# michaelfeil/skyjo_rl

Hardware: AMD Instinct MI355X
Metric: env-steps/sec (whole node) at 65 536 parallel 3-player games (higher is better)
Workload: dtype int8

## Files before the change

### skyjo_rl_amd/csrc/skyjo_capi.hip

```cpp
#include <hip/hip_runtime.h>
#include <hip/hip_ext.h>

#include <cstdio>
#include <cstdlib>
#include <atomic>
#include <cmath>
#include <cstring>
#include <new>
#include <string>
#include <vector>

#include "skyjo_device.h"
#include "skyjo_policy.h"
#include "skyjo_targets.h"
#include "skyjo_batches.h"

#ifdef SK_DIAG
static const char *sk_diag_env(const char *name) { return getenv(name); }
#else
static inline const char *sk_diag_env(const char *) { return nullptr; }
#endif

namespace {

// ... 44 lines not shown
  int cycle_s = 0;
};

enum class InFlight {
  None,
  ListRun,
  Planned,
  Dealing
};

enum class DealRun : int {
  ListBeside = 0,
  ListInline = 1,
  ScanInline = 2,
  Planned = 3
};
constexpr int deal_interval_default(int num_players, DealForm form, int cycle_s) {
  switch (form) {
    case DealForm::OneKernel:
      if (cycle_s >= 4) return num_players >= 3 ? 64 : 56;
      return num_players >= 4 ? 104 : (num_players == 3 ? 80 : 56);
    case DealForm::TwoStreamsPipelined: return num_players >= 3 ? 80 : 56;
    case DealForm::TwoStreamsScanPublish: return num_players >= 3 ? 64 : 48;
    default: return num_players >= 3 ? 88 : 64;
  }
}

}

struct skyjo_vec_mlp {
  SkMlpDev net{};
  void *blob = nullptr;
  int device_id = 0, obs_dim = 0;
};

struct skyjo_vec {
  uint64_t generation = 0;
  skyjo_vec_config cfg{};
  SkParams P{};
  size_t G = 0;
  size_t lds_bytes = 0, lds_tile = 0;
  size_t lds_rollout = 0, lds_step = 0;
  bool seeded = false;
  int pending_iters = 0;
  int deal_every_iters = 64;
  bool auto_interval = true;
  int interval_default = 64, calm_runs = 0;
  uint32_t health_seen = 0;
  uint32_t *health_host = nullptr;
  DealRequests req;
  DealForm form = DealForm::InlineScan;
  bool one_kernel_capable = false;
  int cycle_s = SK_CYCLE_MAX_S;
  size_t lds_cycle = 0, lds_cycle_step = 0;
  uint32_t cycle_deal_arg = 0;
  hipStream_t deal_stream = nullptr;
  hipEvent_t ev_scan = nullptr, ev_dealt = nullptr;
  InFlight inflight = InFlight::None;
  uint32_t inflight_tag = 0;
  int list_sel = 0;
  uint32_t deal_tag = 0;
  uint64_t iter = 0;
  uint64_t iters_total = 0;
  bool fast_host = false, raw_valid = false;
  bool host_spin = true;
  bool raw_export = false;
  uint8_t *hm_block = nullptr;
  int32_t *hm_actions = nullptr;
  uint8_t *hm_mask = nullptr, *hm_records = nullptr, *hm_raw = nullptr;
  int32_t *hm_actions_d = nullptr;
  uint8_t *hm_mask_d = nullptr, *hm_records_d = nullptr, *hm_raw_d = nullptr;
  int raw_stride = 0;
  uint32_t host_seq = 0;
  uint32_t cycle_seq = 0;
  int ncu = 256;
  int max_cycles = 0;
  bool rec_planar_all = false;
  bool rec_planar = false;
  int32_t *d_actions = nullptr;
  uint8_t *d_records = nullptr;
  uint8_t *d_mask = nullptr;
  void *sel_scratch = nullptr;
  size_t sel_blocks = 0;
  std::vector<std::pair<void *, size_t>> allocs;
  std::vector<void *> owned;
  uint8_t *arena = nullptr;
  size_t arena_off = 0;
  int arena_mode = 0;
  bool profile = false;
  std::vector<std::pair<hipEvent_t, hipEvent_t>> ev[SKYJO_PROF_KERNELS];
};

struct skyjo_vec_snapshot {
  const skyjo_vec *owner = nullptr;
  uint64_t owner_generation = 0;
  std::vector<size_t> array_bytes;
  int device_id = 0;
  void *blob = nullptr;
  size_t bytes = 0;
  int pending_iters = 0, deal_every_iters = 0, calm_runs = 0, list_sel = 0;
  bool auto_interval = true;
  uint32_t health_seen = 0, deal_tag = 0, health[2] = {0, 0};
  uint64_t iter = 0, iters_total = 0;
};

namespace {

int dev_error_check(const skyjo_vec *h) {
  if (h->health_host && (h->health_host[2] & SK_ERR_DEAL_TIMEOUT))
    return fail(SKYJO_E_DEVICE, "a step kernel gave up waiting for the dealing kernel that should run beside it (SKYJO_OPT_OVERLAP): "
                                "results since then are void; switch the option off or re-seed");
  return SKYJO_OK;
}

int dev_error_fetch(skyjo_vec *h, hipStream_t s) {
  uint32_t err = 0;
  HIPCHK(hipMemcpyAsync(&err, h->P.dev_error, sizeof(err), hipMemcpyDeviceToHost, s));
  HIPCHK(hipStreamSynchronize(s));
  h->health_host[2] |= err;
  return dev_error_check(h);
}

template <class T>
int dalloc(skyjo_vec *h, T **out, size_t count, bool zero = true) {
  const size_t bytes = count * sizeof(T);
  void *p = nullptr;
  if (h->arena_mode) {
    const size_t al = bytes >= ((size_t)1 << 20) ? ((size_t)2 << 20) : 256;
    const size_t off = (h->arena_off + al - 1) & ~(al - 1);
    h->arena_off = off + bytes;
    if (h->arena_mode == 1) {
      *out = nullptr;
      return SKYJO_OK;
    }
    p = h->arena + off;
  } else {
    HIPCHK(hipMalloc(&p, bytes));
    h->owned.push_back(p);
  }
  if (zero) HIPCHK(hipMemset(p, 0, bytes));
  h->allocs.emplace_back(p, bytes);
  *out = (T *)p;
  return SKYJO_OK;
}

int prof_events(skyjo_vec *h, int kernel, hipEvent_t *a, hipEvent_t *b) {
  *a = *b = nullptr;
  if (!h->profile) return SKYJO_OK;
  HIPCHK(hipEventCreate(a));
  HIPCHK(hipEventCreate(b));
  h->ev[kernel].emplace_back(*a, *b);
  return SKYJO_OK;
}

constexpr uint32_t kDealLds = SK_TILE * (SK_DECK_STRIDE + SK_STG_STRIDE);
constexpr int fixed_players(int n) { return n >= 2 && n <= 4 ? n : 0; }

template <class Fn>
struct KernelRow {
  int key;
  Fn fn;
};
constexpr int kernel_key(int players, bool indirect = false, bool planar = false, bool policy = false) {
  return players | indirect << 4 | planar << 5 | policy << 6;
}
template <class Fn, size_t K>
Fn find_kernel(const KernelRow<Fn> (&table)[K], int key) {
  for (const KernelRow<Fn> &r : table)
    if (r.key == key) return r.fn;
  return nullptr;
}

constexpr KernelRow<decltype(&k_deal<2>)> kDealKernels[] = {{2, k_deal<2>}, {3, k_deal<3>}, {4, k_deal<4>}, {0, k_deal<0>}};

#define SK_ROW(I, NP, PL) {kernel_key(NP, I, PL), k_cycle<I, NP, PL>}
#define SK_ROWS(I, PL) SK_ROW(I, 2, PL), SK_ROW(I, 3, PL), SK_ROW(I, 4, PL)
constexpr KernelRow<decltype(&k_cycle<true, 2, false>)> kCycleKernels[] = {SK_ROWS(true, false), SK_ROWS(true, true), SK_ROWS(false, true), SK_ROWS(false, false)};
#undef SK_ROWS
#undef SK_ROW

#define SK_ROW(I, Pol, NP, PL) {kernel_key(NP, I, PL, Pol), k_step<I, Pol, NP, PL>}
#define SK_ROWS(I, Pol) SK_ROW(I, Pol, 2, false), SK_ROW(I, Pol, 3, false), SK_ROW(I, Pol, 4, false), SK_ROW(I, Pol, 0, false)
constexpr KernelRow<decltype(&k_step<true, true, 2>)> kStepKernels[] = {SK_ROW(true, false, 2, true), SK_ROW(true, false, 3, true), SK_ROW(true, false, 4, true),
                                                                        SK_ROWS(true, true), SK_ROWS(true, false), SK_ROWS(false, true), SK_ROWS(false, false)};
#undef SK_ROWS
#undef SK_ROW

int launch_deal_kernel(skyjo_vec *h, hipStream_t ds, DealRun run, int be_read = -1) {
  hipEvent_t e0, e1;
  int rc;
  h->P.be_read = be_read >= 0 ? (uint32_t)be_read : (h->P.deal_tag & 1u);
  if ((rc = prof_events(h, 2, &e0, &e1))) return rc;
  const int np = fixed_players(h->P.L.N);
  hipExtLaunchKernelGGL(find_kernel(kDealKernels, kernel_key(np)), dim3(h->P.tiles), dim3(SK_TILE), np ? kDealLds : (uint32_t)(h->lds_tile + 16384), ds, e0, e1, 0, h->P,
                        h->list_sel, (int)run);
  HIPCHK(hipGetLastError());
  return SKYJO_OK;
}

int flush_planned(skyjo_vec *h, hipStream_t s) {
  if (h->inflight != InFlight::Planned) return SKYJO_OK;
  const uint32_t keep = h->P.deal_tag;
  h->P.deal_tag = h->inflight_tag;
  h->inflight = InFlight::Dealing;
  const int rc = launch_deal_kernel(h, s, DealRun::Planned, (int)((h->cycle_seq - 1u) & 1u));
  h->P.deal_tag = keep;
  return rc;
}

int publish_deals(skyjo_vec *h, hipStream_t s) {
  int rc = flush_planned(h, s);
  if (rc) return rc;
  if (h->inflight == InFlight::None) return SKYJO_OK;
  if (uses_deal_stream(h->form)) HIPCHK(hipStreamWaitEvent(s, h->ev_dealt, 0));
  hipEvent_t e0, e1;
  if ((rc = prof_events(h, 3, &e0, &e1))) return rc;
  if (h->inflight == InFlight::ListRun) {
    hipExtLaunchKernelGGL(k_publish, dim3(64), dim3(256), 0, s, e0, e1, 0, h->P, h->list_sel);
  } else {
    const int G = h->P.tiles * SK_TILE;
    hipExtLaunchKernelGGL(k_publish_all, dim3((G + 255) / 256), dim3(256), 0, s, e0, e1, 0, h->P);
  }
  HIPCHK(hipGetLastError());
  h->inflight = InFlight::None;
// ... 179 lines not shown
      const char *e = sk_diag_env("SKYJO_OVERLAP");
      one = prefer_one && !e;
      beside = !one && (e ? atoi(e) != 0 : P.tiles <= 768);
    }
  }
  h->form = one      ? DealForm::OneKernel
            : beside ? (h->req.unpipelined ? DealForm::TwoStreamsScanPublish : DealForm::TwoStreamsPipelined)
                     : (h->req.inline_work_list ? DealForm::InlineWorkList : DealForm::InlineScan);
  h->interval_default = deal_interval_default(N, h->form, h->cycle_s);
  if (h->auto_interval) h->deal_every_iters = h->interval_default;
}

int change_form(skyjo_vec *h, const DealRequests &req) {
  HIPCHK(hipDeviceSynchronize());
  int rc = publish_deals(h, nullptr);
  if (rc) return rc;
  HIPCHK(hipDeviceSynchronize());
  h->req = req;
  resolve_form(h);
  return SKYJO_OK;
}

}

extern "C" {

const char *skyjo_vec_last_error(void) { return g_err.c_str(); }
int skyjo_vec_abi_version(void) { return SKYJO_ABI_VERSION; }

int skyjo_vec_create(const skyjo_vec_config *cfg, skyjo_vec **out) {
  if (!cfg || !out) return fail(SKYJO_E_INVALID, "null argument");
  *out = nullptr;
  if (cfg->abi_version != SKYJO_ABI_VERSION) return fail(SKYJO_E_INVALID, "abi_version mismatch");
  if (cfg->num_envs <= 0) return fail(SKYJO_E_INVALID, "num_envs must be > 0");
  if (cfg->num_players <= 0 || cfg->num_players > SKYJO_MAX_PLAYERS)
    return fail(SKYJO_E_INVALID, "Skyjo can be played from 1 up to 8 (recommended) / 12 (theoretical) players");
  if (cfg->rng_mode != SKYJO_RNG_MT19937 && cfg->rng_mode != SKYJO_RNG_PHILOX)
    return fail(SKYJO_E_INVALID, "unknown rng_mode");
  int ndev = 0;
  if (hipGetDeviceCount(&ndev) != hipSuccess || ndev <= 0)
    return fail(SKYJO_E_NOGPU, "no HIP device visible: this library has no CPU fallback");
  if (cfg->device_id < 0 || cfg->device_id >= ndev) return fail(SKYJO_E_INVALID, "device_id out of range");
  hipDeviceProp_t prop;
  HIPCHK(hipGetDeviceProperties(&prop, cfg->device_id));
  if (strncmp(prop.gcnArchName, "gfx950", 6) != 0 && !sk_diag_env("SKYJO_ALLOW_ANY_GPU"))
    return fail(SKYJO_E_NOGPU, std::string("device is ") + prop.gcnArchName + ", kernels are built for gfx950");
  DevGuard guard_(cfg->device_id);

  skyjo_vec *h = new (std::nothrow) skyjo_vec();
  if (!h) return fail(SKYJO_E_INVALID, "out of host memory");
  h->cfg = *cfg;
  h->generation = ++g_generation;
  SkParams &P = h->P;
  P.L = sk_make_layout(cfg->num_players, cfg->observe_indirect);
  P.B = cfg->num_envs;
  P.tiles = (cfg->num_envs + SK_TILE - 1) / SK_TILE;
  P.rng_mode = cfg->rng_mode;
  P.auto_reset = cfg->auto_reset ? 1 : 0;
  P.score_penalty = cfg->score_penalty, P.mean_reward = cfg->mean_reward;
  P.reward_refunded = cfg->reward_refunded, P.illegal_reward = cfg->illegal_reward;
  P.game_id0 = cfg->game_id0;
  P.spin_log2 = 22, P.debug_deal_delay = 0;
  h->G = (size_t)P.tiles * SK_TILE;
  h->lds_tile = (size_t)P.L.chunks * 1024;
  h->lds_bytes = h->lds_tile + (size_t)SK_TILE * (P.L.indirect ? 64 : P.L.rec_bytes + 16) + (size_t)SK_ACC_KINDS * cfg->num_players * 512 +
                 (cfg->num_players < 8 ? (size_t)cfg->num_players * 1024 : 0);
  const bool fixed_n = cfg->num_players >= 2 && cfg->num_players <= 4;
  h->lds_step = fixed_n ? h->lds_tile + (size_t)SK_TILE * (P.L.indirect ? 64 : P.L.rec_bytes + 16) : h->lds_bytes;
  h->lds_rollout = fixed_n ? h->lds_step + (size_t)cfg->num_players * 1024 : h->lds_bytes;
  if (const char *e = sk_diag_env("SKYJO_LDS_PAD"))
    h->lds_bytes += (size_t)atoi(e), h->lds_rollout += (size_t)atoi(e), h->lds_step += (size_t)atoi(e);
  const size_t rec16 = (size_t)P.tiles * P.L.chunks * SK_TILE;
  if ((uint64_t)SK_BANK * rec16 * 16 >= (1ull << 32)) {
    delete h;
    return fail(SKYJO_E_INVALID, "num_envs too large for one handle");
  }
  int rc = SKYJO_OK;
  const size_t N = (size_t)cfg->num_players;
  auto carve = [&]() -> int {
    int rc = SKYJO_OK;
    if (cfg->rng_mode == SKYJO_RNG_MT19937 && (rc = dalloc(h, &P.mt, h->G * 624 + 16, false)  )) {
      return rc;
    }
    if ((rc = dalloc(h, &P.state, rec16)) || (rc = dalloc(h, &P.spare, SK_BANK * rec16)) ||
        (rc = dalloc(h, &P.spare_ready, SK_BANK * h->G)) || (rc = dalloc(h, &P.bank_head, h->G)) ||
        (rc = dalloc(h, &P.busy, h->G)) || (rc = dalloc(h, &P.cancel, h->G)) || (rc = dalloc(h, &P.done_flag, h->G)) || (rc = dalloc(h, &P.plan_tag, h->G)) || (rc = dalloc(h, &P.plan_ep, h->G)) ||
        (rc = dalloc(h, &P.deal_list, 2 * h->G)) || (rc = dalloc(h, &P.deal_ep, 2 * h->G)) ||
        (rc = dalloc(h, &P.deal_count, 2)) || (rc = dalloc(h, &P.bank_empty, 2)) ||
        (rc = dalloc(h, &P.mt_idx, (1 + SK_BANK) * h->G)) || (rc = dalloc(h, &P.seeds, h->G)) ||
        (rc = dalloc(h, &P.deals_consumed, h->G)) || (rc = dalloc(h, &P.rewards, h->G * N)) ||
        (rc = dalloc(h, &P.scores, h->G * N)) || (rc = dalloc(h, &P.done, h->G)) ||
        (rc = dalloc(h, &P.acc_tile, (size_t)P.tiles * SK_ACC_KINDS * SKYJO_MAX_PLAYERS)) || (rc = dalloc(h, &P.dev_error, 1)) ||
        (rc = dalloc(h, &P.counters, 1)) || (rc = dalloc(h, &P.tile_counters, (size_t)P.tiles * 8)) || (rc = dalloc(h, &P.stamps, (size_t)P.tiles * 32))) {
      return rc;
    }
    return SKYJO_OK;
  };
  h->arena_mode = 1, h->arena_off = 0;
  (void)carve();
  {
    const size_t two_mb = (size_t)2 << 20, total = h->arena_off + two_mb;
    void *raw = nullptr;
    if (hipMalloc(&raw, total) != hipSuccess) {
      skyjo_vec_destroy(h);
      return fail(SKYJO_E_DEVICE, "hipMalloc failed for the engine's arrays");
    }
    h->owned.push_back(raw);
    h->arena = (uint8_t *)(((uintptr_t)raw + two_mb - 1) & ~(uintptr_t)(two_mb - 1));
  }
  h->arena_mode = 2, h->arena_off = 0;
  rc = carve();
  h->arena_mode = 0;
  if (rc) {
    skyjo_vec_destroy(h);
    return rc;
  }
  int prio_least = 0, prio_greatest = 0;
  (void)hipDeviceGetStreamPriorityRange(&prio_least, &prio_greatest);
  if (hipStreamCreateWithPriority(&h->deal_stream, hipStreamNonBlocking, prio_least) != hipSuccess ||
      hipEventCreateWithFlags(&h->ev_scan, hipEventDisableTiming) != hipSuccess ||
      hipEventCreateWithFlags(&h->ev_dealt, hipEventDisableTiming) != hipSuccess) {
    skyjo_vec_destroy(h);
    return fail(SKYJO_E_DEVICE, "cannot create the dealing stream / events");
  }
  {
    void *dp = nullptr;
    if (hipHostMalloc((void **)&h->health_host, 4 * sizeof(uint32_t), hipHostMallocMapped) != hipSuccess ||
        hipHostGetDevicePointer(&dp, h->health_host, 0) != hipSuccess) {
      skyjo_vec_destroy(h);
      return fail(SKYJO_E_DEVICE, "cannot map the bank-health word");
    }
    h->health_host[0] = h->health_host[1] = h->health_host[2] = h->health_host[3] = 0;
    P.health_host = (volatile uint32_t *)dp;
  }
  h->raw_stride = (int)((P.L.state_bytes + 16 * cfg->num_players + 8 + 15) & ~15);
  if (h->G <= 4096) {
    const size_t a = (h->G * 4 + 255) & ~(size_t)255, m = (h->G + 255) & ~(size_t)255, r = (h->G * (size_t)P.L.rec_bytes + 255) & ~(size_t)255,
                 w = h->G * (size_t)h->raw_stride;
    void *dp = nullptr;
    if (hipHostMalloc((void **)&h->hm_block, a + m + r + w, hipHostMallocMapped) == hipSuccess &&
        hipHostGetDevicePointer(&dp, h->hm_block, 0) == hipSuccess) {
      memset(h->hm_block, 0, a + m + r + w);
      uint8_t *d = (uint8_t *)dp;
      h->hm_actions = (int32_t *)h->hm_block, h->hm_mask = h->hm_block + a, h->hm_records = h->hm_block + a + m, h->hm_raw = h->hm_block + a + m + r;
      h->hm_actions_d = (int32_t *)d, h->hm_mask_d = d + a, h->hm_records_d = d + a + m, h->hm_raw_d = d + a + m + r;
      h->fast_host = !sk_diag_env("SKYJO_NO_FAST_HOST");
      h->host_spin = !sk_diag_env("SKYJO_NO_SPIN");
      h->raw_export = h->fast_host && P.tiles <= 4 && !sk_diag_env("SKYJO_NO_RAW_EXPORT");
    }
  }
  h->ncu = prop.multiProcessorCount > 0 ? prop.multiProcessorCount : 256;
  if (const char *e = sk_diag_env("SKYJO_FUSED_SCAN")) h->req.inline_work_list = atoi(e) == 0;
  if (const char *e = sk_diag_env("SKYJO_PIPELINED")) h->req.unpipelined = atoi(e) == 0;
  resolve_form(h);
  if (const char *e = sk_diag_env("SKYJO_DEAL_INTERVAL")) {
    const int v = atoi(e);
    if (v >= 1 && v <= 1024) h->deal_every_iters = v, h->auto_interval = false;
  }
  *out = h;
  return SKYJO_OK;
}

int skyjo_vec_destroy(skyjo_vec *h) {
  if (!h) return SKYJO_OK;
  GUARD(h);
  (void)hipDeviceSynchronize();
  if (h->deal_stream) (void)hipStreamDestroy(h->deal_stream);
  if (h->ev_scan) (void)hipEventDestroy(h->ev_scan);
  if (h->ev_dealt) (void)hipEventDestroy(h->ev_dealt);
  for (void *p : h->owned) (void)hipFree(p);
  if (h->sel_scratch) (void)hipFree(h->sel_scratch);
  for (auto &v : h->ev)
    for (auto &e : v) (void)hipEventDestroy(e.first), (void)hipEventDestroy(e.second);
  if (h->health_host) (void)hipHostFree(h->health_host);
  if (h->hm_block) (void)hipHostFree(h->hm_block);
  delete h;
  return SKYJO_OK;
}

int skyjo_vec_get_info(const skyjo_vec *h, skyjo_vec_info *out) {
  if (!h || !out) return fail(SKYJO_E_INVALID, "null argument");
  const SkLayout &L = h->P.L;
  out->num_envs = h->P.B, out->num_players = L.N, out->obs_dim = L.D, out->record_bytes = L.rec_bytes;
  out->mask_offset = L.Dp, out->meta_offset = L.Dp + 26, out->state_bytes = L.state_bytes, out->tile_games = SK_TILE;
  return SKYJO_OK;
}

int skyjo_vec_seed(skyjo_vec *h, const uint64_t *seeds_host, uint64_t base_seed, void *stream) {
  if (!h) return fail(SKYJO_E_INVALID, "null handle");
  hipStream_t s = (hipStream_t)stream;
  GUARD(h);
  h->raw_valid = false;
  uint64_t *d_seeds = nullptr;
  if (seeds_host) {
    HIPCHK(hipMalloc((void **)&d_seeds, sizeof(uint64_t) * (size_t)h->P.B));
    HIPCHK(hipMemcpyAsync(d_seeds, seeds_host, sizeof(uint64_t) * (size_t)h->P.B, hipMemcpyHostToDevice, s));
  }
  HIPCHK(hipDeviceSynchronize());
  HIPCHK(hipMemsetAsync(h->P.done, 0, h->G, s));
  HIPCHK(hipMemsetAsync(h->P.dev_error, 0, sizeof(uint32_t), s));
  h->health_host[2] = 0;
  int rc0;
  if ((rc0 = publish_deals(h, s))) return rc0;
  hipLaunchKernelGGL(k_seed, dim3((h->P.B + 255) / 256), dim3(256), 0, s, h->P, (const uint64_t *)d_seeds, base_seed, 0,
                     h->P.B);
  HIPCHK(hipGetLastError());
  int rc;
  h->inflight = InFlight::None;
  if ((rc = start_deals(h, s)) || (rc = publish_deals(h, s))) return rc;
  h->seeded = true;
  if ((rc = skyjo_vec_reset(h, nullptr, nullptr, stream))) return rc;
  for (int k = 1; k < SK_BANK; k++)
    if ((rc = start_deals(h, s)) || (rc = publish_deals(h, s))) return rc;
  if (d_seeds) {
    HIPCHK(hipStreamSynchronize(s));
    HIPCHK(hipFree(d_seeds));
  }
  h->iter = 0;
  return skyjo_vec_reset_counters(h, stream);
}

static int ensure_scratch(skyjo_vec *h);

int skyjo_vec_seed_one(skyjo_vec *h, int32_t game, uint64_t value, void *stream) {
  if (!h || game < 0 || game >= h->P.B) return fail(SKYJO_E_INVALID, "bad argument");
  if (!h->seeded) return fail(SKYJO_E_STATE, "skyjo_vec_seed must be called first");
  GUARD(h);
  h->raw_valid = false;
  hipStream_t s = (hipStream_t)stream;
  int rc;
  if ((rc = ensure_scratch(h)) || (rc = publish_deals(h, s))) return rc;
  uint64_t *d_seed = (uint64_t *)h->d_actions;
  HIPCHK(hipMemcpyAsync(d_seed, &value, sizeof(value), hipMemcpyHostToDevice, s));
  HIPCHK(hipStreamSynchronize(s));
  hipLaunchKernelGGL(k_seed, dim3(1), dim3(64), 0, s, h->P, (const uint64_t *)d_seed, (uint64_t)0, (int)game, 1);
  HIPCHK(hipGetLastError());
  if ((rc = start_deals(h, s)) || (rc = publish_deals(h, s))) return rc;
  HIPCHK(hipMemsetAsync(h->d_mask, 0, h->G, s));
  const uint8_t one = 1;
  HIPCHK(hipMemcpyAsync(h->d_mask + game, &one, 1, hipMemcpyHostToDevice, s));
  HIPCHK(hipStreamSynchronize(s));
  if ((rc = skyjo_vec_reset(h, h->d_mask, nullptr, stream))) return rc;
  for (int k = 1; k < SK_BANK; k++)
    if ((rc = start_deals(h, s)) || (rc = publish_deals(h, s))) return rc;
  return SKYJO_OK;
}

int skyjo_vec_snapshot_create(skyjo_vec *h, skyjo_vec_snapshot **out, void *stream) {
  if (!h || !out) return fail(SKYJO_E_INVALID, "null argument");
  if (!h->seeded) return fail(SKYJO_E_STATE, "skyjo_vec_seed must be called first");
  GUARD(h);
  hipStream_t s = (hipStream_t)stream;
  int rc;
  if ((rc = publish_deals(h, s))) return rc;
  HIPCHK(hipDeviceSynchronize());
  if ((rc = dev_error_fetch(h, s))) return rc;
  skyjo_vec_snapshot *sn = new (std::nothrow) skyjo_vec_snapshot();
  if (!sn) return fail(SKYJO_E_INVALID, "out of host memory");
  sn->owner = h, sn->owner_generation = h->generation, sn->device_id = h->cfg.device_id;
  for (auto &a : h->allocs) sn->bytes += (a.second + 255) & ~(size_t)255, sn->array_bytes.push_back(a.second);
  if (hipMalloc(&sn->blob, sn->bytes) != hipSuccess) {
    delete sn;
    return fail(SKYJO_E_DEVICE, "hipMalloc failed for the snapshot");
  }
  size_t off = 0;
  for (auto &a : h->allocs) {
    hipError_t e = hipMemcpyAsync((uint8_t *)sn->blob + off, a.first, a.second, hipMemcpyDeviceToDevice, s);
    if (e != hipSuccess) {
      (void)hipFree(sn->blob);
      delete sn;
      return fail(SKYJO_E_DEVICE, std::string("snapshot copy: ") + hipGetErrorString(e));
    }
    off += (a.second + 255) & ~(size_t)255;
  }
  if (hipError_t e = hipStreamSynchronize(s); e != hipSuccess) {
    (void)hipFree(sn->blob);
    delete sn;
    return fail(SKYJO_E_DEVICE, std::string("snapshot copy: ") + hipGetErrorString(e));
  }
  sn->pending_iters = h->pending_iters, sn->deal_every_iters = h->deal_every_iters, sn->calm_runs = h->calm_runs;
  sn->list_sel = h->list_sel, sn->auto_interval = h->auto_interval, sn->health_seen = h->health_seen;
  sn->deal_tag = h->deal_tag, sn->iter = h->iter, sn->iters_total = h->iters_total;
  sn->health[0] = h->health_host[0], sn->health[1] = h->health_host[1];
  *out = sn;
  return SKYJO_OK;
}

int skyjo_vec_snapshot_restore(skyjo_vec *h, const skyjo_vec_snapshot *sn, void *stream) {
  if (!h || !sn) return fail(SKYJO_E_INVALID, "null argument");
  if (sn->owner != h || sn->owner_generation != h->generation)
    return fail(SKYJO_E_INVALID, "the snapshot was taken from another handle");
  if (sn->array_bytes.size() > h->allocs.size()) return fail(SKYJO_E_INVALID, "the snapshot does not fit the handle's arrays");
  for (size_t k = 0; k < sn->array_bytes.size(); k++)
    if (sn->array_bytes[k] != h->allocs[k].second) return fail(SKYJO_E_INVALID, "the snapshot does not fit the handle's arrays");
  GUARD(h);
  hipStream_t s = (hipStream_t)stream;
  int rc;
  if ((rc = publish_deals(h, s))) return rc;
  HIPCHK(hipDeviceSynchronize());
  size_t off = 0;
  for (size_t k = 0; k < sn->array_bytes.size(); k++) {
    const auto &a = h->allocs[k];
    HIPCHK(hipMemcpyAsync(a.first, (const uint8_t *)sn->blob + off, a.second, hipMemcpyDeviceToDevice, s));
    off += (a.second + 255) & ~(size_t)255;
  }
  HIPCHK(hipStreamSynchronize(s));
  h->pending_iters = sn->pending_iters, h->deal_every_iters = sn->deal_every_iters, h->calm_runs = sn->calm_runs;
  h->list_sel = sn->list_sel, h->auto_interval = sn->auto_interval, h->health_seen = sn->health_seen;
  h->deal_tag = sn->deal_tag, h->P.deal_tag = sn->deal_tag, h->iter = sn->iter, h->iters_total = sn->iters_total;
  h->health_host[0] = sn->health[0], h->health_host[1] = sn->health[1];
  h->health_host[2] = 0;
  h->inflight = InFlight::None;
  h->raw_valid = false;
  return SKYJO_OK;
}

int skyjo_vec_snapshot_bytes(const skyjo_vec_snapshot *sn, size_t *bytes_out) {
  if (!sn || !bytes_out) return fail(SKYJO_E_INVALID, "null argument");
  *bytes_out = sn->bytes;
  return SKYJO_OK;
}

int skyjo_vec_snapshot_destroy(skyjo_vec_snapshot *sn) {
  if (!sn) return SKYJO_OK;
  DevGuard guard_(sn->device_id);
  (void)hipFree(sn->blob);
  delete sn;
  return SKYJO_OK;
}

static int reset_impl(skyjo_vec *h, const uint8_t *mask, void *records_out, hipStream_t s, uint8_t *raw_out, int planar = 0) {
  int rc;
  h->raw_valid = false;
  if ((rc = publish_deals(h, s))) return rc;
  dim3 grid(h->P.tiles), block(SK_TILE);
  if (h->P.L.indirect)
    hipLaunchKernelGGL((k_reset<true>), grid, block, h->lds_bytes, s, h->P, mask, (uint8_t *)records_out, raw_out, h->raw_stride, planar);
  else
    hipLaunchKernelGGL((k_reset<false>), grid, block, h->lds_bytes, s, h->P, mask, (uint8_t *)records_out, raw_out, h->raw_stride, 0);
  HIPCHK(hipGetLastError());
  if ((rc = start_deals(h, s))) return rc;
  return publish_deals(h, s);
}

int skyjo_vec_reset(skyjo_vec *h, const uint8_t *mask, void *records_out, void *stream) {
  if (!h) return fail(SKYJO_E_INVALID, "null handle");
  GUARD(h);
  if (!h->seeded) return fail(SKYJO_E_STATE, "skyjo_vec_seed must be called first");
  return reset_impl(h, mask, records_out, (hipStream_t)stream, nullptr, h->rec_planar_all ? 1 : 0);
}

static int step_once(skyjo_vec *h, const int32_t *actions, void *records_out, double *end_rew, uint8_t *end_flag, hipStream_t s,
                     uint8_t *raw_out = nullptr, bool planar_out = false) {
  const bool due = h->pending_iters + 1 >= h->deal_every_iters;
  if (due && plans_ahead(h)) plan_cycle(h);
  int rc = launch_step(h, s, false, actions, (uint8_t *)records_out, nullptr, 1, 0, end_rew, end_flag, raw_out, 0, planar_out && records_out);
  if (rc) return rc;
  return due ? start_due_deals(h, s) : SKYJO_OK;
}

int skyjo_vec_step(skyjo_vec *h, const int32_t *actions, void *records_out, void *stream) {
  if (!h || !actions) return fail(SKYJO_E_INVALID, "null argument");
  GUARD(h);
  if (!h->seeded) return fail(SKYJO_E_STATE, "skyjo_vec_seed must be called first");
  return step_once(h, actions, records_out, nullptr, nullptr, (hipStream_t)stream, nullptr, h->rec_planar_all);
}

int skyjo_vec_step_collect(skyjo_vec *h, const int32_t *actions, void *records_out, double *final_rewards_out,
                           uint8_t *episode_end_out, void *stream) {
  if (!h || !actions || !final_rewards_out || !episode_end_out) return fail(SKYJO_E_INVALID, "null argument");
  GUARD(h);
  if (!h->seeded) return fail(SKYJO_E_STATE, "skyjo_vec_seed must be called first");
  return step_once(h, actions, records_out, final_rewards_out, episode_end_out, (hipStream_t)stream, nullptr, h->rec_planar_all);
}

static int model_check(skyjo_vec *h, const skyjo_vec_mlp *policy, const skyjo_vec_mlp *value, int32_t T, const skyjo_vec_rollout_buffers *b) {
  if (!h || !policy || !b || T < 0 || !b->records || !b->actions) return fail(SKYJO_E_INVALID, "skyjo_vec_model_rollout: bad argument");
  if (value && !b->values) return fail(SKYJO_E_INVALID, "skyjo_vec_model_rollout: a value net needs a values buffer");
  if ((b->final_rewards == nullptr) != (b->episode_end == nullptr))
    return fail(SKYJO_E_INVALID, "skyjo_vec_model_rollout: final_rewards and episode_end go together");
  if (!h->seeded) return fail(SKYJO_E_STATE, "skyjo_vec_seed must be called first");
  if (policy->net.out_dim != SKYJO_NUM_ACTIONS) return fail(SKYJO_E_INVALID, "the policy net needs 26 outputs");
  if (policy->device_id != h->cfg.device_id || policy->obs_dim != h->P.L.D || !h->P.L.indirect)
    return fail(SKYJO_E_INVALID, "the policy net must live on the engine's device and take the engine's (indirect) observation");
  if (value && (policy->obs_dim != value->obs_dim || policy->device_id != value->device_id || policy->net.split != value->net.split))
    return fail(SKYJO_E_INVALID, "policy and value net must share the observation size, the precision and the device");
  return SKYJO_OK;
}
// ... 31 lines not shown
}

int skyjo_vec_rollout(skyjo_vec *h, int32_t iters, uint64_t policy_seed, void *records_out, int32_t *actions_out,
                      void *stream) {
  if (!h || iters < 0) return fail(SKYJO_E_INVALID, "bad argument");
  GUARD(h);
  if (!h->seeded) return fail(SKYJO_E_STATE, "skyjo_vec_seed must be called first");
  hipStream_t s = (hipStream_t)stream;
  uint8_t *rec = (uint8_t *)records_out;
  const bool planar = h->rec_planar;
  if (planar && rec && h->form != DealForm::OneKernel)
    return fail(SKYJO_E_STATE, "SKYJO_OPT_RECORD_LAYOUT = tile-planar needs the one-kernel dealing form (SKYJO_OPT_OVERLAP 3)");
  for (int done = 0; done < iters;) {
    int n = iters - done < kMaxRolloutChunk ? iters - done : kMaxRolloutChunk;
    const int due = h->deal_every_iters - h->pending_iters;
    if (n > due) n = due > 0 ? due : 1;
    const bool run_due = h->pending_iters + n >= h->deal_every_iters, planned = plans_ahead(h);
    int cycles = 1;
    if (h->form == DealForm::OneKernel && planned && run_due && h->pending_iters == 0) {
      const int cap = h->max_cycles > 0 ? h->max_cycles : kMaxCyclesPerLaunch;
      cycles = (iters - done) / h->deal_every_iters;
      cycles = cycles < 1 ? 1 : (cycles > cap ? cap : cycles);
      n = cycles * h->deal_every_iters;
    }
    if (run_due && planned) {
      plan_cycle(h);
      const uint32_t first = h->deal_tag;
      for (int c = 1; c < cycles; c++) next_deal_tag(h, false);
      h->P.plan_new_tag = first;
    }
    int rc = launch_step(h, s, true, nullptr, rec, actions_out, n, policy_seed, nullptr, nullptr, nullptr, cycles > 1 ? h->deal_every_iters : 0);
    if (rc) return rc;
    done += n;
    if (run_due && (rc = start_due_deals(h, s))) return rc;
    if (rec) rec += (size_t)n * (planar ? h->G : (size_t)h->P.B) * h->P.L.rec_bytes;
    if (actions_out) actions_out += (size_t)n * h->P.B;
  }
  return SKYJO_OK;
}

static int observe_impl(skyjo_vec *h, const int32_t *players, void *records_out, void *stream, int planar) {
  if (!h || !records_out) return fail(SKYJO_E_INVALID, "null argument");
  GUARD(h);
  if (!h->seeded) return fail(SKYJO_E_STATE, "skyjo_vec_seed must be called first");
  dim3 grid(h->P.tiles), block(SK_TILE);
  hipStream_t s = (hipStream_t)stream;
  if (h->P.L.indirect)
    hipLaunchKernelGGL((k_observe<true>), grid, block, h->lds_bytes, s, h->P, players, (uint8_t *)records_out, planar);
  else
    hipLaunchKernelGGL((k_observe<false>), grid, block, h->lds_bytes, s, h->P, players, (uint8_t *)records_out, 0);
  HIPCHK(hipGetLastError());
  return SKYJO_OK;
}
int skyjo_vec_observe(skyjo_vec *h, const int32_t *players, void *records_out, void *stream) {
  return observe_impl(h, players, records_out, stream, h && h->rec_planar_all ? 1 : 0);
}

static int unpack_impl(skyjo_vec *h, const void *records, int64_t n, int8_t *obs, int8_t *mask, uint8_t *agent, uint8_t *phase, uint8_t *done,
                       uint8_t *status, void *stream, int planar) {
  if (!h || !records || n < 0) return fail(SKYJO_E_INVALID, "bad argument");
  GUARD(h);
  if (n == 0) return SKYJO_OK;
  long long total = n * (long long)(h->P.L.D + 26);
  int blocks = (int)((total + 255) / 256);
  if (blocks > 4096) blocks = 4096;
  hipLaunchKernelGGL(k_unpack, dim3(blocks), dim3(256), 0, (hipStream_t)stream, h->P.L, (const uint8_t *)records,
                     (long long)n, obs, mask, agent, phase, done, status, planar);
  HIPCHK(hipGetLastError());
  return SKYJO_OK;
}

int skyjo_vec_unpack(skyjo_vec *h, const void *records, int64_t n, int8_t *obs, int8_t *mask, uint8_t *agent,
                     uint8_t *phase, uint8_t *done, uint8_t *status, void *stream) {
  return unpack_impl(h, records, n, obs, mask, agent, phase, done, status, stream, 0);
}

int skyjo_vec_unpack_tiles(skyjo_vec *h, const void *records, int64_t n_tiles, int8_t *obs, int8_t *mask, uint8_t *agent,
                           uint8_t *phase, uint8_t *done, uint8_t *status, void *stream) {
  return unpack_impl(h, records, n_tiles * SK_TILE, obs, mask, agent, phase, done, status, stream, 1);
}

const double *skyjo_vec_rewards_ptr(const skyjo_vec *h) { return h ? h->P.rewards : nullptr; }
const double *skyjo_vec_scores_ptr(const skyjo_vec *h) { return h ? h->P.scores : nullptr; }
const uint8_t *skyjo_vec_done_ptr(const skyjo_vec *h) { return h ? h->P.done : nullptr; }

int skyjo_vec_sample_actions_layout(skyjo_vec *h, const void *records, int32_t layout, const float *logits, int64_t n, uint64_t seed,
                                    uint64_t ticket, int32_t no_masking, int32_t *actions_out, float *logp_out,
                                    float *uniform_out, void *stream) {
  if (!h || !records || !logits || !actions_out || n < 0) return fail(SKYJO_E_INVALID, "null argument");
  if (layout != SKYJO_REC_ROW_MAJOR && layout != SKYJO_REC_TILE_PLANAR) return fail(SKYJO_E_INVALID, "layout must be SKYJO_REC_ROW_MAJOR or SKYJO_REC_TILE_PLANAR");
  GUARD(h);
  if (n == 0) return SKYJO_OK;
  const int64_t blocks = (n + SK_SAMPLE_BLOCK - 1) / SK_SAMPLE_BLOCK;
  hipLaunchKernelGGL(k_sample, dim3((unsigned)blocks), dim3(SK_SAMPLE_BLOCK), 0, (hipStream_t)stream, h->P.L,
                     (const uint8_t *)records, logits, (long long)n, seed, ticket, h->P.game_id0, (int)no_masking,
                     actions_out, logp_out, uniform_out, (int)(layout == SKYJO_REC_TILE_PLANAR));
  HIPCHK(hipGetLastError());
  return SKYJO_OK;
}
int skyjo_vec_sample_actions(skyjo_vec *h, const void *records, const float *logits, int64_t n, uint64_t seed,
                             uint64_t ticket, int32_t no_masking, int32_t *actions_out, float *logp_out,
                             float *uniform_out, void *stream) {
  return skyjo_vec_sample_actions_layout(h, records, SKYJO_REC_ROW_MAJOR, logits, n, seed, ticket, no_masking, actions_out, logp_out, uniform_out,
                                         stream);
}

int skyjo_vec_mlp_create(int32_t device_id, int32_t obs_dim, int32_t out_dim, int32_t precision, const float *w1, const float *b1,
                         const float *w2, const float *b2, const float *w3, const float *b3, skyjo_vec_mlp **out) {
  if (!out || !w1 || !b1 || !w2 || !b2 || !w3 || !b3) return fail(SKYJO_E_INVALID, "null argument");
  if (obs_dim < 1 || obs_dim > SKP_IN - 1 || out_dim < 1 || out_dim > SKP_OUT)
    return fail(SKYJO_E_INVALID, "skyjo_vec_mlp: obs_dim must be 1..31 and out_dim 1..32");
  if (precision != SKYJO_MLP_BF16 && precision != SKYJO_MLP_FP32) return fail(SKYJO_E_INVALID, "skyjo_vec_mlp: unknown precision");
  int ndev = 0;
  if (hipGetDeviceCount(&ndev) != hipSuccess || device_id < 0 || device_id >= ndev) return fail(SKYJO_E_INVALID, "device_id out of range");
  DevGuard guard_(device_id);
  auto bf16 = [](float f) {
    uint32_t u;
    memcpy(&u, &f, 4);
    u += 0x7fffu + ((u >> 16) & 1u);
    return (uint16_t)(u >> 16);
  };
  auto bf16_to_float = [](uint16_t b) {
    const uint32_t u = (uint32_t)b << 16;
    float f;
    memcpy(&f, &u, 4);
    return f;
  };
  auto bf16_lo = [&](float f) {
    const uint32_t hi = (uint32_t)bf16(f) << 16;
    float fh;
    memcpy(&fh, &hi, 4);
    return bf16(f - fh);
  };
  const bool split = precision == SKYJO_MLP_FP32;
  auto acc_k = [](int ks, int hh, int j) { return 32 * (ks >> 1) + 16 * (ks & 1) + 8 * (j >> 2) + 4 * hh + (j & 3); };
  const int H = SKP_HIDDEN;
  const size_t e1 = (size_t)8 * 2 * 64 * 8, e2 = (size_t)8 * 16 * 64 * 8, e3 = (size_t)16 * 64 * 8;
  std::vector<uint16_t> f1(e1), f2(e2), f3(e3), g1(split ? e1 : 0), g2(split ? e2 : 0), g3(split ? e3 : 0);
  std::vector<float> c2((size_t)H), c3((size_t)64 * 16);
  for (int u = 0; u < 8; u++)
    for (int l = 0; l < 64; l++) {
      const int m = 32 * u + (l & 31), hh = l >> 5;
      for (int s = 0; s < 2; s++)
        for (int j = 0; j < 8; j++) {
          const int k = 16 * s + 8 * hh + j;
          const float v = SKP_SCALE * (k < obs_dim ? w1[(size_t)m * obs_dim + k] : (k == SKP_IN - 1 ? b1[m] : 0.f));
          const size_t at = (((size_t)u * 2 + s) * 64 + l) * 8 + j;
          f1[at] = bf16(v);
          if (split) g1[at] = bf16_lo(v);
        }
      for (int ks = 0; ks < 16; ks++)
        for (int j = 0; j < 8; j++) {
          const float v = SKP_SCALE * w2[(size_t)m * H + acc_k(ks, hh, j)];
          const size_t at = (((size_t)u * 16 + ks) * 64 + l) * 8 + j;
          f2[at] = split ? bf16(v) : bf16(-2.0f * v);
          if (split) g2[at] = bf16_lo(v);
        }
    }
  for (int l = 0; l < 64; l++) {
    const int m = l & 31, hh = l >> 5;
    for (int ks = 0; ks < 16; ks++)
      for (int j = 0; j < 8; j++) {
        const float v = m < out_dim ? w3[(size_t)m * H + acc_k(ks, hh, j)] : 0.f;
        const size_t at = ((size_t)ks * 64 + l) * 8 + j;
        f3[at] = split ? bf16(v) : bf16(-2.0f * v);
        if (split) g3[at] = bf16_lo(v);
      }
// ... 269 lines not shown
int skyjo_vec_get_state(skyjo_vec *h, int32_t game, skyjo_game_state *o, void *stream) {
  if (!h || !o || game < 0 || game >= h->P.B) return fail(SKYJO_E_INVALID, "bad argument");
  GUARD(h);
  hipStream_t s = (hipStream_t)stream;
  const SkLayout &L = h->P.L;
  if (h->raw_valid) {
    const uint8_t *raw = h->hm_raw + (size_t)game * h->raw_stride;
    decode_state(L, raw, o);
    const double *d = (const double *)(raw + L.state_bytes);
    if (o->done) {
      memcpy(o->rewards, d, sizeof(double) * L.N);
      if (o->is_terminated) memcpy(o->final_score, d + L.N, sizeof(double) * L.N);
    }
    return dev_error_check(h);
  }
  std::vector<uint8_t> r;
  int rc = fetch_record(h, h->P.state, game, r, s);
  if (rc) return rc;
  decode_state(L, r.data(), o);
  if (o->done) {
    HIPCHK(hipMemcpyAsync(o->rewards, h->P.rewards + (size_t)game * L.N, sizeof(double) * L.N, hipMemcpyDeviceToHost, s));
    if (o->is_terminated)
      HIPCHK(hipMemcpyAsync(o->final_score, h->P.scores + (size_t)game * L.N, sizeof(double) * L.N,
                            hipMemcpyDeviceToHost, s));
    HIPCHK(hipStreamSynchronize(s));
  }
  return dev_error_check(h);
}

int skyjo_vec_set_state(skyjo_vec *h, int32_t game, const skyjo_game_state *in, void *stream) {
  if (!h || !in || game < 0 || game >= h->P.B) return fail(SKYJO_E_INVALID, "bad argument");
  GUARD(h);
  if (!h->seeded) return fail(SKYJO_E_STATE, "skyjo_vec_seed must be called first");
  h->raw_valid = false;
  const SkLayout &L = h->P.L;
  if (in->n_draw < 0 || in->n_disc < 0 || in->n_draw + in->n_disc > SK_NCARDS)
    return fail(SKYJO_E_INVALID, "pile sizes out of range");
  if (in->expected_player >= L.N || in->expected_phase > 1) return fail(SKYJO_E_INVALID, "bad expected action");
  hipStream_t s = (hipStream_t)stream;
  std::vector<uint8_t> r((size_t)L.state_bytes, 0);
  int ms = 1 << 30, mh = 1 << 30;
  for (int p = 0; p < L.N; p++) {
    int sum = 0, hid = 0;
    for (int k = 0; k < 12; k++) {
      int8_t c = in->players_cards[p][k];
      int m = in->players_masked[p][k];
      if (c < -2 && !(m == 0 && c == SKYJO_REFUNDED)) return fail(SKYJO_E_INVALID, "card value out of range");
      if (c > 12) return fail(SKYJO_E_INVALID, "card value out of range");
      int8_t v = m == 2 ? (int8_t)SKYJO_HAND_NONE : (m == 0 ? (int8_t)SKYJO_REFUNDED : c);
      r[sk_pb(L, p) + PB_CARDS + k] = (uint8_t)(m == 0 ? (int8_t)SKYJO_REFUNDED : c);
      r[sk_pb(L, p) + PB_VIS + k] = (uint8_t)v;
      if (m == 1) {
        sum += c;
        if (!L.indirect) r[H_HIST + 2 + c]++;
      }
      if (m == 2) hid++;
    }
    int16_t s16 = (int16_t)sum;
    memcpy(&r[sk_pb(L, p) + PB_SUM], &s16, 2);
    r[sk_pb(L, p) + PB_HIDDEN] = (uint8_t)hid;
    r[sk_pb(L, p) + PB_REFUNDED] = (uint8_t)in->num_refunded[p];
    uint16_t pl = (uint16_t)in->num_placed[p];
    memcpy(&r[sk_pb(L, p) + PB_PLACED], &pl, 2);
    ms = sum < ms ? sum : ms, mh = hid < mh ? hid : mh;
  }
  for (int k = 0; k < in->n_draw; k++) r[L.off_pile + k] = (uint8_t)in->drawpile[k];
  for (int k = 0; k < in->n_disc; k++) {
    int8_t c = in->discard_pile[k];
    if (c < -2 || c > 12) return fail(SKYJO_E_INVALID, "discard value out of range");
    r[L.off_pile + SK_NCARDS - 1 - k] = (uint8_t)c;
    r[H_HIST + 2 + c]++;
  }
  r[H_PHASE] = in->expected_phase, r[H_PLAYER] = in->expected_player;
  r[H_FLAGS] = F_VALID | (in->is_terminated ? (F_TERMINATED | F_DONE) : 0) | (in->done ? F_DONE : 0);
  r[H_STATUS] = in->status;
  r[H_NDRAW] = (uint8_t)in->n_draw, r[H_NDISC] = (uint8_t)in->n_disc, r[H_ROLE] = 0;
  memcpy(&r[H_EPLEN], &in->episode_steps, 2);
  r[H_RESH] = (uint8_t)(in->reshuffles > 255 ? 255 : in->reshuffles);
  memcpy(&r[H_EPISODE], &in->episode, 4);
  r[H_MINSUM] = (uint8_t)(int8_t)(ms < 127 ? ms : 127);
  r[H_MINHID] = (uint8_t)mh;
  r[H_TOP] = in->n_disc ? (uint8_t)in->discard_pile[in->n_disc - 1] : (uint8_t)(int8_t)-3;
  r[H_HAND] = (uint8_t)in->hand_card;
  HIPCHK(hipMemcpyAsync(&r[H_BANK], h->P.bank_head + game, 1, hipMemcpyDeviceToHost, s));
  HIPCHK(hipStreamSynchronize(s));
  uint8_t *dst = (uint8_t *)(h->P.state + ((size_t)(game / SK_TILE) * L.chunks) * SK_TILE + game % SK_TILE);
  HIPCHK(hipMemcpy2DAsync(dst, SK_TILE * 16, r.data(), 16, 16, L.chunks, hipMemcpyHostToDevice, s));
  uint8_t dn = (r[H_FLAGS] & F_DONE) ? 1 : 0;
  HIPCHK(hipMemcpyAsync(h->P.done + game, &dn, 1, hipMemcpyHostToDevice, s));
  if (dn) {
    HIPCHK(hipMemcpyAsync(h->P.rewards + (size_t)game * L.N, in->rewards, sizeof(double) * L.N, hipMemcpyHostToDevice, s));
    HIPCHK(hipMemcpyAsync(h->P.scores + (size_t)game * L.N, in->final_score, sizeof(double) * L.N,
                          hipMemcpyHostToDevice, s));
  }
  HIPCHK(hipStreamSynchronize(s));
  return SKYJO_OK;
}

int skyjo_vec_seed_raw(skyjo_vec *h, int32_t game, uint32_t value, void *stream) {
  if (!h || game < 0 || game >= h->P.B) return fail(SKYJO_E_INVALID, "bad argument");
  GUARD(h);
  if (!h->seeded) return fail(SKYJO_E_STATE, "skyjo_vec_seed must be called first");
  if (h->P.rng_mode != SKYJO_RNG_MT19937) return fail(SKYJO_E_STATE, "seed_raw needs the MT19937 mode");
  h->raw_valid = false;
  hipStream_t s = (hipStream_t)stream;
  int rc;
  if ((rc = publish_deals(h, s))) return rc;
  hipLaunchKernelGGL(k_seed_raw, dim3(1), dim3(64), 0, s, h->P, game, value);
  HIPCHK(hipGetLastError());
  if ((rc = start_deals(h, s))) return rc;
  return publish_deals(h, s);
}

int skyjo_vec_rng_set_state(skyjo_vec *h, int32_t game, const uint32_t *key_host, int32_t pos, void *stream) {
  if (!h || !key_host || game < 0 || game >= h->P.B || pos < 0 || pos > 624) return fail(SKYJO_E_INVALID, "bad argument");
  GUARD(h);
  if (!h->seeded) return fail(SKYJO_E_STATE, "skyjo_vec_seed must be called first");
  if (h->P.rng_mode != SKYJO_RNG_MT19937 || !h->req.no_bank)
    return fail(SKYJO_E_STATE, "skyjo_vec_rng_set_state needs the MT19937 mode and SKYJO_OPT_NO_BANK (episodes dealt ahead would belong to the old stream)");
  hipStream_t s = (hipStream_t)stream;
  const int32_t packed = pos >= 624 ? 0 : (pos | ((624 - pos) << 16));
  HIPCHK(hipMemcpyAsync(h->P.mt + (size_t)game * 624, key_host, 624 * sizeof(uint32_t), hipMemcpyHostToDevice, s));
  HIPCHK(hipMemcpyAsync(h->P.mt_idx + game, &packed, sizeof(packed), hipMemcpyHostToDevice, s));
  HIPCHK(hipStreamSynchronize(s));
  return SKYJO_OK;
}

int skyjo_vec_rng_get_state(skyjo_vec *h, int32_t game, uint32_t *key_out_host, int32_t *pos_out_host, void *stream) {
  if (!h || !key_out_host || !pos_out_host || game < 0 || game >= h->P.B) return fail(SKYJO_E_INVALID, "bad argument");
  GUARD(h);
  if (!h->seeded) return fail(SKYJO_E_STATE, "skyjo_vec_seed must be called first");
  if (h->P.rng_mode != SKYJO_RNG_MT19937 || !h->req.no_bank)
    return fail(SKYJO_E_STATE, "skyjo_vec_rng_get_state needs the MT19937 mode and SKYJO_OPT_NO_BANK");
  hipStream_t s = (hipStream_t)stream;
  int32_t packed = 0;
  HIPCHK(hipMemcpyAsync(key_out_host, h->P.mt + (size_t)game * 624, 624 * sizeof(uint32_t), hipMemcpyDeviceToHost, s));
  HIPCHK(hipMemcpyAsync(&packed, h->P.mt_idx + game, sizeof(packed), hipMemcpyDeviceToHost, s));
  HIPCHK(hipStreamSynchronize(s));
  int idx = packed & 0xffff, ahead = packed >> 16;
  if (idx >= 624) idx = 0;
  if (idx + ahead > 624) return fail(SKYJO_E_STATE, "the stream's regenerated window wraps: not a numpy state (cannot happen without a bank)");
  if (idx == 0 && ahead == 0) {
    *pos_out_host = 624;
    return SKYJO_OK;
  }
  uint32_t *mt = key_out_host;
  for (int i = idx + ahead; i < 624; i++) {
    const uint32_t y = (mt[i] & 0x80000000u) | (mt[i + 1 == 624 ? 0 : i + 1] & 0x7fffffffu);
    mt[i] = mt[i + 397 >= 624 ? i + 397 - 624 : i + 397] ^ (y >> 1) ^ ((y & 1u) ? 0x9908b0dfu : 0u);
  }
  *pos_out_host = idx;
  return SKYJO_OK;
}

int skyjo_vec_profile(skyjo_vec *h, int enable, double ms_out[SKYJO_PROF_KERNELS], int64_t launches_out[SKYJO_PROF_KERNELS]) {
  if (!h) return fail(SKYJO_E_INVALID, "null handle");
  GUARD(h);
  HIPCHK(hipDeviceSynchronize());
  for (int k = 0; k < SKYJO_PROF_KERNELS; k++) {
    double tot = 0;
    int64_t cnt = 0;
    for (auto &p : h->ev[k]) {
      float ms = 0.f;
      if (hipEventElapsedTime(&ms, p.first, p.second) == hipSuccess) tot += ms, cnt++;
      (void)hipEventDestroy(p.first);
      (void)hipEventDestroy(p.second);
    }
    h->ev[k].clear();
    if (ms_out) ms_out[k] = tot;
    if (launches_out) launches_out[k] = cnt;
  }
  h->profile = enable != 0;
// ... 115 lines not shown
    h->P.host_seq = 0;
    if (rc) return rc;
    bool arrived = false;
    if (spin) {
      const volatile uint32_t *flag = h->health_host + 3;
      for (long k = 0; k < 4000000 && !(arrived = __atomic_load_n(flag, __ATOMIC_ACQUIRE) == h->host_seq); k++) __builtin_ia32_pause();
    }
    if (!arrived) HIPCHK(hipStreamSynchronize(nullptr));
    h->raw_valid = h->raw_export;
    if (records_out_host) memcpy(records_out_host, h->hm_records, (size_t)h->P.B * h->P.L.rec_bytes);
    return dev_error_check(h);
  }
  int rc = ensure_scratch(h);
  if (rc) return rc;
  HIPCHK(hipMemcpy(h->d_actions, actions_host, sizeof(int32_t) * (size_t)h->P.B, hipMemcpyHostToDevice));
  if ((rc = skyjo_vec_step(h, h->d_actions, h->d_records, nullptr))) return rc;
  if (records_out_host)
    HIPCHK(hipMemcpy(records_out_host, h->d_records, (size_t)h->P.B * h->P.L.rec_bytes, hipMemcpyDeviceToHost));
  else
    HIPCHK(hipStreamSynchronize(nullptr));
  return dev_error_check(h);
}

int skyjo_vec_observe_host(skyjo_vec *h, const int32_t *players_host, void *records_out_host) {
  if (!h || !records_out_host) return fail(SKYJO_E_INVALID, "null argument");
  GUARD(h);
  if (h->fast_host) {
    if (players_host) memcpy(h->hm_actions, players_host, sizeof(int32_t) * (size_t)h->P.B);
    int rc = observe_impl(h, players_host ? h->hm_actions_d : nullptr, h->hm_records_d, nullptr, 0);
    if (rc) return rc;
    HIPCHK(hipStreamSynchronize(nullptr));
    memcpy(records_out_host, h->hm_records, (size_t)h->P.B * h->P.L.rec_bytes);
    return dev_error_check(h);
  }
  int rc = ensure_scratch(h);
  if (rc) return rc;
  if (players_host)
    HIPCHK(hipMemcpy(h->d_actions, players_host, sizeof(int32_t) * (size_t)h->P.B, hipMemcpyHostToDevice));
  if ((rc = observe_impl(h, players_host ? h->d_actions : nullptr, h->d_records, nullptr, 0))) return rc;
  HIPCHK(hipMemcpy(records_out_host, h->d_records, (size_t)h->P.B * h->P.L.rec_bytes, hipMemcpyDeviceToHost));
  return dev_error_check(h);
}

int skyjo_vec_reset_host(skyjo_vec *h, const uint8_t *mask_host, void *records_out_host) {
  if (!h) return fail(SKYJO_E_INVALID, "null handle");
  GUARD(h);
  if (!h->seeded) return fail(SKYJO_E_STATE, "skyjo_vec_seed must be called first");
  if (h->fast_host) {
    if (mask_host) memcpy(h->hm_mask, mask_host, (size_t)h->P.B);
    int rc = reset_impl(h, mask_host ? h->hm_mask_d : nullptr, h->hm_records_d, nullptr, h->raw_export ? h->hm_raw_d : nullptr);
    if (rc) return rc;
    HIPCHK(hipStreamSynchronize(nullptr));
    h->raw_valid = h->raw_export;
    if (records_out_host) memcpy(records_out_host, h->hm_records, (size_t)h->P.B * h->P.L.rec_bytes);
    return dev_error_check(h);
  }
  int rc = ensure_scratch(h);
  if (rc) return rc;
  if (mask_host) HIPCHK(hipMemcpy(h->d_mask, mask_host, (size_t)h->P.B, hipMemcpyHostToDevice));
  if ((rc = skyjo_vec_reset(h, mask_host ? h->d_mask : nullptr, h->d_records, nullptr))) return rc;
  if (records_out_host)
    HIPCHK(hipMemcpy(records_out_host, h->d_records, (size_t)h->P.B * h->P.L.rec_bytes, hipMemcpyDeviceToHost));
  else
    HIPCHK(hipStreamSynchronize(nullptr));
  return dev_error_check(h);
}

int skyjo_vec_get_rewards_host(skyjo_vec *h, double *rewards_out, double *scores_out, uint8_t *done_out) {
  if (!h) return fail(SKYJO_E_INVALID, "null handle");
  GUARD(h);
  const size_t n = (size_t)h->P.B * h->P.L.N;
  if (h->raw_valid) {
    const size_t N = (size_t)h->P.L.N;
    for (int g = 0; g < h->P.B; g++) {
      const uint8_t *raw = h->hm_raw + (size_t)g * h->raw_stride + h->P.L.state_bytes;
      if (rewards_out) memcpy(rewards_out + g * N, raw, 8 * N);
      if (scores_out) memcpy(scores_out + g * N, raw + 8 * N, 8 * N);
      if (done_out) done_out[g] = raw[16 * N + 4];
    }
    return dev_error_check(h);
  }
  if (rewards_out) HIPCHK(hipMemcpy(rewards_out, h->P.rewards, n * sizeof(double), hipMemcpyDeviceToHost));
  if (scores_out) HIPCHK(hipMemcpy(scores_out, h->P.scores, n * sizeof(double), hipMemcpyDeviceToHost));
  if (done_out) HIPCHK(hipMemcpy(done_out, h->P.done, (size_t)h->P.B, hipMemcpyDeviceToHost));
  return dev_error_check(h);
}

int skyjo_dev_malloc(int device_id, size_t bytes, void **out) {
  if (!out) return fail(SKYJO_E_INVALID, "null argument");
  DevGuard guard_(device_id);
  HIPCHK(hipMalloc(out, bytes ? bytes : 1));
  return SKYJO_OK;
}
int skyjo_dev_free(void *p) {
  if (p) HIPCHK(hipFree(p));
  return SKYJO_OK;
}
namespace {
struct DevBuf {
  void *p = nullptr;
  ~DevBuf() {
    if (p) (void)hipFree(p);
  }
};
int score_device(int32_t device_id, int *ndev_out) {
  int ndev = 0;
  if (hipGetDeviceCount(&ndev) != hipSuccess || ndev <= 0) return fail(SKYJO_E_NOGPU, "no HIP device visible: this library has no CPU fallback");
  if (device_id < 0 || device_id >= ndev) return fail(SKYJO_E_INVALID, "device_id out of range");
  *ndev_out = ndev;
  return SKYJO_OK;
}
}

int skyjo_vec_evaluate_game(int32_t device_id, int32_t n, int32_t num_players, const int8_t *players_cards_host, const int32_t *player_won_id_host,
                        double score_penalty, double *scores_out_host) {
  if (!players_cards_host || !player_won_id_host || !scores_out_host || n < 0) return fail(SKYJO_E_INVALID, "skyjo_vec_evaluate_game: bad argument");
  if (num_players <= 0 || num_players > SKYJO_MAX_PLAYERS) return fail(SKYJO_E_INVALID, "skyjo_vec_evaluate_game: num_players must be 1..12");
  for (int32_t i = 0; i < n; i++)
    if (player_won_id_host[i] < 0 || player_won_id_host[i] >= num_players) return fail(SKYJO_E_INVALID, "skyjo_vec_evaluate_game: player_won_id out of range");
  int ndev, rc;
  if ((rc = score_device(device_id, &ndev))) return rc;
  if (n == 0) return SKYJO_OK;
  DevGuard guard_(device_id);
  const size_t cb = (size_t)n * num_players * 12, wb = (size_t)n * 4, sb = (size_t)n * num_players * 8;
  const size_t o_w = (cb + 255) & ~(size_t)255, o_s = o_w + ((wb + 255) & ~(size_t)255);
  DevBuf d;
  HIPCHK(hipMalloc(&d.p, o_s + sb));
  uint8_t *b = (uint8_t *)d.p;
  HIPCHK(hipMemcpy(b, players_cards_host, cb, hipMemcpyHostToDevice));
  HIPCHK(hipMemcpy(b + o_w, player_won_id_host, wb, hipMemcpyHostToDevice));
  hipLaunchKernelGGL(k_evaluate_game, dim3((n + 63) / 64), dim3(64), 0, nullptr, (int)n, (int)num_players, (const int8_t *)b, (const int32_t *)(b + o_w),
                     score_penalty, (double *)(b + o_s));
  HIPCHK(hipGetLastError());
  HIPCHK(hipMemcpy(scores_out_host, b + o_s, sb, hipMemcpyDeviceToHost));
  return SKYJO_OK;
}

int skyjo_vec_calc_final_rewards(int32_t device_id, int32_t n, int32_t num_players, const double *final_score_host, const int32_t *num_refunded_host,
                             double mean_reward, double reward_refunded, double *rewards_out_host) {
  if (!final_score_host || !num_refunded_host || !rewards_out_host || n < 0) return fail(SKYJO_E_INVALID, "skyjo_vec_calc_final_rewards: bad argument");
  if (num_players <= 0 || num_players > SKYJO_MAX_PLAYERS) return fail(SKYJO_E_INVALID, "skyjo_vec_calc_final_rewards: num_players must be 1..12");
  int ndev, rc;
  if ((rc = score_device(device_id, &ndev))) return rc;
  if (n == 0) return SKYJO_OK;
  DevGuard guard_(device_id);
  const size_t sb = (size_t)n * num_players * 8, fb = (size_t)n * num_players * 4;
  const size_t o_f = (sb + 255) & ~(size_t)255, o_r = o_f + ((fb + 255) & ~(size_t)255);
  DevBuf d;
  HIPCHK(hipMalloc(&d.p, o_r + sb));
  uint8_t *b = (uint8_t *)d.p;
  HIPCHK(hipMemcpy(b, final_score_host, sb, hipMemcpyHostToDevice));
  HIPCHK(hipMemcpy(b + o_f, num_refunded_host, fb, hipMemcpyHostToDevice));
  hipLaunchKernelGGL(k_final_rewards, dim3((n + 63) / 64), dim3(64), 0, nullptr, (int)n, (int)num_players, (const double *)b, (const int32_t *)(b + o_f),
                     mean_reward, reward_refunded, (double *)(b + o_r));
  HIPCHK(hipGetLastError());
  HIPCHK(hipMemcpy(rewards_out_host, b + o_r, sb, hipMemcpyDeviceToHost));
  return SKYJO_OK;
}

int skyjo_dev_copy(void *dst, const void *src, size_t bytes, int kind, void *stream) {
  hipMemcpyKind k = kind == 1 ? hipMemcpyHostToDevice : kind == 2 ? hipMemcpyDeviceToHost : hipMemcpyDeviceToDevice;
  HIPCHK(hipMemcpyAsync(dst, src, bytes, k, (hipStream_t)stream));
  if (kind == 2) HIPCHK(hipStreamSynchronize((hipStream_t)stream));
  return SKYJO_OK;
}
int skyjo_dev_sync(void *stream) {
  HIPCHK(hipStreamSynchronize((hipStream_t)stream));
// ... 5 lines not shown
```

### skyjo_rl_amd/csrc/skyjo_deal.h

```cpp
#pragma once
#ifndef SKYJO_DEVICE_PARTS
#error "include skyjo_device.h"
#endif

__global__ void k_seed(SkParams P, const uint64_t *seeds, uint64_t base, int first, int count) {
  const int i = blockIdx.x * blockDim.x + threadIdx.x;
  if (i >= count) return;
  const int g = first + i;
  const uint64_t value = seeds ? seeds[i] : base + P.game_id0 + (uint64_t)g;
  const size_t G = (size_t)P.tiles * SK_TILE;
  P.seeds[g] = value;
  P.deals_consumed[g] = 0;
  for (int k = 0; k < SK_BANK; k++) P.spare_ready[(size_t)k * G + g] = 0;
  P.bank_head[g] = 0, P.busy[g] = 0, P.cancel[g] = 0, P.done_flag[g] = 0;
  if (P.rng_mode == SKYJO_RNG_MT19937) {
    uint32_t *mt = P.mt + (size_t)g * 624;
    uint32_t x = (uint32_t)(value + 1);
    mt[0] = x;
    for (int k = 1; k < 624; k++) {
      x = 1812433253u * (x ^ (x >> 30)) + (uint32_t)k;
      mt[k] = x;
    }
    P.mt_idx[g] = 0;
  }
}

__global__ void k_seed_raw(SkParams P, int g, uint32_t value) {
  if (threadIdx.x != 0 || blockIdx.x != 0) return;
  uint32_t *mt = P.mt + (size_t)g * 624;
  uint32_t x = value;
  mt[0] = x;
  for (int k = 1; k < 624; k++) {
    x = 1812433253u * (x ^ (x >> 30)) + (uint32_t)k;
    mt[k] = x;
  }
  P.mt_idx[g] = 0;
  const size_t G = (size_t)P.tiles * SK_TILE;
  for (int k = 0; k < SK_BANK; k++) P.spare_ready[(size_t)k * G + g] = 0;
}

template <class Rng>
__device__ __forceinline__ void shuffle_lds(uint8_t *lp, int base, int n, Rng &r) {
  int i = n - 1;
  if (i < 1) return;
  uint32_t mask = 0xffffffffu >> __clz(i);
  r.service();
  uint32_t pre = r.next();
  while (i >= 1) {
    const uint32_t v = pre & mask;
    r.service();
    pre = r.next();
    if (v <= (uint32_t)i) {
      const uint8_t t = LB(base + i);
      LB(base + i) = LB(base + (int)v), LB(base + (int)v) = t;
      i--;
      mask = 0xffffffffu >> __clz(i | 1);
    }
  }
  r.unget();
}

#define SK_SHUFFLE_STEP(q)                                                                        \
  if (i >= 1) {                                                                                   \
    const uint32_t v = (q) & mask;                                                                \
    r.rp++, r.used++;                                                                             \
    if (v <= (uint32_t)i) {                                                                       \
      const int bv = base + (int)v, bi = base + i;                                                \
      const uint8_t av = LB(bv);                                                                  \
      LB(bi) = av, LB(bv) = (uint8_t)ai;                                                          \
      i--;                                                                                        \
      mask = 0xffffffffu >> __clz(i | 1);                                                         \
      ai = LB(base + i);                                                                          \
    }                                                                                             \
  }
__device__ __forceinline__ void shuffle_lds(uint8_t *lp, int base, int n, MtStream<64> &r) {
  int i = n - 1;
  if (i < 1) return;
  uint8_t *fp = r.fp;
  uint32_t mask = 0xffffffffu >> __clz(i);
  int ai = LB(base + i);
  while (__any(i >= 1)) {
    r.service(16);
#pragma unroll 1
    for (int grp = 0; grp < 4; grp++) {
      const uint32_t q0 = MT_FIFO(r.rp & 63), q1 = MT_FIFO((r.rp + 1) & 63), q2 = MT_FIFO((r.rp + 2) & 63),
                     q3 = MT_FIFO((r.rp + 3) & 63);
      SK_SHUFFLE_STEP(q0)
      SK_SHUFFLE_STEP(q1)
      SK_SHUFFLE_STEP(q2)
      SK_SHUFFLE_STEP(q3)
    }
  }
}

#define SK_STG_STRIDE 80
struct MtChunkStream {
  uint32_t *mt;
  int base, pos, gen, chunks_made;
  uint32_t R[16], o[17], x[16], xw;
  static constexpr bool kLockstep = true;
  uint32_t *mt0;
  uint32_t my_off;
  uint8_t *stg;
  int lane;
  __device__ __forceinline__ static int wrap(int v) { return v >= 624 ? v - 624 : v; }
  __device__ __forceinline__ void open(uint32_t *mt0_, uint32_t my_off_, int packed, uint8_t *stg_, int lane_) {
    mt0 = mt0_, my_off = my_off_, mt = mt0_ + my_off_, stg = stg_, lane = lane_, chunks_made = 0;
    int idx = packed & 0xffff;
    idx = idx >= 624 ? 0 : idx;
    const int ahead = packed >> 16;
    gen = wrap(idx + ahead);
    base = gen == 0 ? 608 : gen - 16;
    pos = 16 - ahead;
    if (ahead > 0) {
#pragma unroll
      for (int k = 0; k < 16; k++) R[k] = mt_temper(mt[base + k]);
    }
  }
  __device__ __forceinline__ int close() const { return wrap(base + pos) | (((16 - pos) & 31) << 16); }
  __device__ __forceinline__ void issue() {
    const int c = gen;
// ... 259 lines not shown
  for (int d = 0; d < (SK_NCARDS + 3) / 4; d++) {
    uint32_t m = 0;
    for (int j = 0; j < 4; j++)
      if (4 * d + j < R - 1) m |= 0xffu << (8 * j);
    uint32_t w = m ? (pack4(12 * NP + 4 * d) & m) : 0u;
    if (d == (SK_NCARDS - 1) / 4) w |= ((uint32_t)last & 0xffu) << (((SK_NCARDS - 1) & 3) * 8);
    rec[(H_PILE >> 2) + d] |= w;
  }
  rec[0] = (uint32_t)best << 8 | (uint32_t)F_VALID << 16 | (uint32_t)SKYJO_ST_RESET << 24;
  rec[1] = (uint32_t)(R - 1) | 1u << 8 | ((uint32_t)last & 0xffu) << 24;
  rec[2] = (uint32_t)SKYJO_HAND_NONE << 24;
  rec[3] = episode;
  setb(H_MINSUM, (uint32_t)(ms < 127 ? ms : 127)), setb(H_MINHID, 10);
#pragma unroll
  for (int c = 0; c < 20; c++)
    if (4 * c < nwords) dst[c] = make_uint4(rec[4 * c], rec[4 * c + 1], rec[4 * c + 2], rec[4 * c + 3]);
}
#undef DKW

template <class Rng>
__device__ __forceinline__ void deal_into_lds(const SkParams &P, uint8_t *lp, Rng &r, uint32_t episode) {
  const int N = P.L.N, pb = P.L.off_pile, R = SK_NCARDS - 12 * N;
  const int pw = pb >> 2;
  const int tmp = pb + R;
  for (int c = 0; c < P.L.chunks; c++) LQ(c) = make_uint4(0u, 0u, 0u, 0u);
  for (int d = 0; d < (SK_NCARDS + 3) / 4; d++) {
    uint32_t w = 0;
    for (int j = 0; j < 4; j++) {
      const int i = 4 * d + j;
      w |= (i < SK_NCARDS ? (uint32_t)((-2 + i / 10) & 0xff) : 0u) << (8 * j);
    }
    LW(pw + d) = w;
  }
#pragma unroll 1
  for (int seg = 0; seg < N + 2; seg++) {
    int base = pb, n = SK_NCARDS;
    if (seg == 1) {
      for (int p = 0; p < N; p++)
        for (int j = 0; j < 3; j++) LW((sk_pb(P.L, p) >> 2) + j) = LW(pw + 3 * p + j);
      for (int d = 0; d < (R + 3) / 4; d += 8) {
        uint32_t t[8];
#pragma unroll
        for (int k = 0; k < 8; k++) t[k] = LW(pw + 3 * N + d + k);
#pragma unroll
        for (int k = 0; k < 8; k++)
          if (d + k < (R + 3) / 4) LW(pw + d + k) = t[k];
      }
      n = R;
    } else if (seg >= 2) {
      const int p = seg - 2;
      for (int k = 0; k < 12; k++) LB(tmp + k) = (uint8_t)k, LB(sk_pb(P.L, p) + PB_VIS + k) = SKYJO_HAND_NONE;
      base = tmp, n = 12;
    }
    shuffle_lds(lp, base, n, r);
    if (seg >= 2) {
      const int p = seg - 2;
      int s0 = LB(tmp), s1 = LB(tmp + 1);
      const int blk = sk_pb(P.L, p);
      int c0 = LI(blk + PB_CARDS + s0), c1 = LI(blk + PB_CARDS + s1);
      LB(blk + PB_VIS + s0) = (uint8_t)c0, LB(blk + PB_VIS + s1) = (uint8_t)c1;
      LSH(blk + PB_SUM) = (int16_t)(c0 + c1);
      LB(blk + PB_HIDDEN) = 10;
      if (!P.L.indirect) LB(H_HIST + 2 + c0)++, LB(H_HIST + 2 + c1)++;
    }
  }
  for (int k = R; k < SK_NCARDS; k++) LB(pb + k) = 0;
  const int last = LI(pb + R - 1);
  LB(pb + R - 1) = 0;
  LB(pb + SK_NCARDS - 1) = (uint8_t)last;
  LB(H_HIST + 2 + last)++;
  int best = 0, bs = LSH(sk_pb(P.L, 0) + PB_SUM);
  for (int p = 1; p < N; p++) {
    int s = LSH(sk_pb(P.L, p) + PB_SUM);
    if (s > bs) bs = s, best = p;
  }
  LB(H_PHASE) = 0, LB(H_PLAYER) = (uint8_t)best, LB(H_FLAGS) = F_VALID, LB(H_STATUS) = SKYJO_ST_RESET;
  LB(H_NDRAW) = (uint8_t)(R - 1), LB(H_NDISC) = 1, LB(H_ROLE) = 0;
  LB(H_TOP) = (uint8_t)last, LB(H_HAND) = SKYJO_HAND_NONE;
  *(uint32_t *)(lp + LIDX(H_EPISODE)) = episode;
  refresh_minima(P, lp);
}

__device__ __forceinline__ bool deal_inline(const SkParams &P, uint8_t *lp, uint8_t *fp, int g, int tile, int lane, int head) {
  const uint32_t ep = P.deals_consumed[g];
  const int busy = P.busy[g];
  if (busy) {
    const bool cancelled = P.cancel[g] != 0;
    if (P.rng_mode == SKYJO_RNG_MT19937 && !cancelled) {
      const int w = wait_deal_done(P, g);
      if (w == SK_WAIT_TIMEOUT) {
        LB(H_FLAGS) = F_VALID | F_DONE, LB(H_STATUS) = SKYJO_ST_ERROR;
        for (int q = 0; q < P.L.N; q++) P.rewards[(size_t)g * P.L.N + q] = 0.0;
        return false;
      }
      P.cancel[g] = 1;
      if (w == SK_WAIT_OK) {
        load_spare(P, lp, busy - 1, tile, lane);
        bank_advance(P, lp, g, head, ep);
        return true;
      }
    }
    P.cancel[g] = 1;
  }
  if (P.rng_mode == SKYJO_RNG_MT19937) {
    MtStream<16> r;
    r.open(P.mt + (size_t)g * 624, P.mt_idx[g], fp);
    deal_into_lds(P, lp, r, ep);
    P.mt_idx[g] = r.close();
  } else {
    PhiloxStream r;
    r.open(P.seeds[g] + 1, ep, 0u, 0u);
    deal_into_lds(P, lp, r, ep);
  }
  LB(H_BANK) = (uint8_t)head;
  P.deals_consumed[g] = ep + 1;
  P.done[g] = 0;
  return true;
}

#define SK_SCAN_BLOCK 1024
__global__ __launch_bounds__(SK_SCAN_BLOCK) void k_scan(SkParams P, int list_sel) {
  __shared__ uint32_t wave_need[SK_SCAN_BLOCK / 64], block_first;
  const size_t G = (size_t)P.tiles * SK_TILE;
  const int lane = threadIdx.x & 63, wave = threadIdx.x >> 6;
  int32_t *list = P.deal_list + (size_t)list_sel * G;
  uint32_t *eps = P.deal_ep + (size_t)list_sel * G;
  for (int base = blockIdx.x * SK_SCAN_BLOCK; base < P.B; base += gridDim.x * SK_SCAN_BLOCK) {
    const int g = base + (int)threadIdx.x;
    bool need = false;
    int slot = 0, r = 0;
    uint32_t consumed = 0;
    if (g < P.B) {
      const uint8_t busy = P.busy[g];
      const int head = P.bank_head[g] % SK_BANK;
      consumed = P.deals_consumed[g];
      uint8_t ready[SK_BANK];
#pragma unroll
      for (int k = 0; k < SK_BANK; k++) ready[k] = P.spare_ready[(size_t)k * G + g];
      bool open = true;
#pragma unroll
      for (int k = 0; k < SK_BANK; k++) {
        uint8_t f = 0;
#pragma unroll
        for (int j = 0; j < SK_BANK; j++) f = (head + k) % SK_BANK == j ? ready[j] : f;
        open = open && f != 0;
        r += open ? 1 : 0;
      }
      need = !busy && r < SK_BANK;
      slot = (head + r) % SK_BANK;
    }
    const unsigned long long b = __ballot(need);
    const unsigned long long be = __ballot(need && r == 0);
    if (lane == 0) {
      wave_need[wave] = (uint32_t)__popcll(b);
      if (be) atomicAdd(P.bank_empty, (uint32_t)__popcll(be));
    }
    __syncthreads();
    if (threadIdx.x == 0) {
      uint32_t total = 0;
      for (int w = 0; w < SK_SCAN_BLOCK / 64; w++) {
        const uint32_t n = wave_need[w];
        wave_need[w] = total;
        total += n;
      }
      block_first = total ? atomicAdd(&P.deal_count[list_sel], total) : 0u;
    }
    __syncthreads();
    if (need) {
      const uint32_t pos = block_first + wave_need[wave] + (uint32_t)__popcll(b & ((1ull << lane) - 1ull));
      list[pos] = g;
      eps[pos] = consumed + (uint32_t)r;
      P.busy[g] = (uint8_t)(1 + slot);
      P.cancel[g] = 0;
      P.plan_tag[g] = P.deal_tag;
    }
    __syncthreads();
  }
}

__global__ __launch_bounds__(256) void k_publish(SkParams P, int list_sel) {
  const size_t G = (size_t)P.tiles * SK_TILE;
  const int32_t *list = P.deal_list + (size_t)list_sel * G;
  const int count = (int)P.deal_count[list_sel];
  if (blockIdx.x == 0 && threadIdx.x == 0) {
    P.deal_count[list_sel ^ 1] = 0;
    P.health_host[0] = *P.bank_empty, P.health_host[1] = P.deal_tag;
    *P.bank_empty = 0;
  }
  for (int i = blockIdx.x * blockDim.x + threadIdx.x; i < count; i += gridDim.x * blockDim.x) {
    const int g = list[i];
    const int slot = P.busy[g] - 1;
    if (slot >= 0 && !P.cancel[g] && P.done_flag[g] == P.deal_tag) P.spare_ready[(size_t)slot * G + g] = 1;
    P.busy[g] = 0, P.cancel[g] = 0;
  }
}

__global__ __launch_bounds__(256) void k_publish_all(SkParams P) {
  const int g = blockIdx.x * blockDim.x + threadIdx.x;
  if (g < P.tiles * SK_TILE) sk_publish_deals(P, g);
}

template <int NP>
__device__ __forceinline__ void deal_body(const SkParams &P, int list_sel, int publish_inline, const int block, const int lane, uint32_t *lds_raw,
                                          const bool report_health = true) {
  TRACE_DECL;
  uint8_t *lp = (uint8_t *)lds_raw + lane * 16;
  const size_t G = (size_t)P.tiles * SK_TILE;
  const int count = (int)P.deal_count[list_sel];
  const int i = block * SK_TILE + lane;
  const bool fused = publish_inline == 2, piped = publish_inline == 3;
  if (piped && report_health && block == 0 && lane == 0) {
    uint32_t *be = P.bank_empty + (P.be_read & 1u);
    P.health_host[0] = *be, P.health_host[1] = P.deal_tag;
    *be = 0;
  }
  if (!piped && publish_inline && block == 0 && lane == 0) {
    P.deal_count[list_sel ^ 1] = 0;
    uint32_t *be = P.bank_empty + (fused ? (list_sel ^ 1) & 1 : 0);
    P.health_host[0] = *be, P.health_host[1] = P.deal_tag;
    *be = 0;
  }
  if (!fused && !piped && block * SK_TILE >= count) return;
  for (uint32_t k = 0; k < P.debug_deal_delay; k++) __builtin_amdgcn_s_sleep(127);
  const int tile = block;
  (void)tile;
  STAMP_DECL;
  STAMP(0);
  int g, slot;
  uint32_t ep;
  bool act;
  if (fused) {
    const bool listed = i < P.B;
    g = listed ? i : 0;
    const uint8_t busy = P.busy[g];
    const int head = P.bank_head[g] % SK_BANK;
    const uint32_t consumed = P.deals_consumed[g];
    uint8_t ready[SK_BANK];
#pragma unroll
    for (int k = 0; k < SK_BANK; k++) ready[k] = P.spare_ready[(size_t)k * G + g];
    bool open = true;
    int r = 0;
#pragma unroll
    for (int k = 0; k < SK_BANK; k++) {
      uint8_t f = 0;
#pragma unroll
      for (int j = 0; j < SK_BANK; j++) f = (head + k) % SK_BANK == j ? ready[j] : f;
      open = open && f != 0;
      r += open ? 1 : 0;
    }
    act = listed && !busy && r < SK_BANK;
    slot = (head + r) % SK_BANK;
    ep = consumed + (uint32_t)r;
    const unsigned long long be = __ballot(act && r == 0);
    if (be && lane == 0) atomicAdd(P.bank_empty + (list_sel & 1), (uint32_t)__popcll(be));
  } else if (piped) {
    const bool listed = i < P.B;
    g = listed ? i : 0;
    const int owner = listed ? P.busy[g] : 0;
    act = owner > 0 && P.plan_tag[g] == P.deal_tag;
    slot = act ? owner - 1 : 0;
    ep = P.plan_ep[g];
  } else {
    const bool listed = i < count;
    g = listed ? P.deal_list[(size_t)list_sel * G + i] : 0;
    ep = listed ? P.deal_ep[(size_t)list_sel * G + i] : 0u;
    const int owner = listed ? P.busy[g] : 0;
    act = owner > 0;
    slot = act ? owner - 1 : 0;
  }
  uint4 *dst = P.spare + bank_rec16(P, slot, g);
  bool mt_overrun = false;
  if (P.rng_mode == SKYJO_RNG_MT19937) {
    const int packed = P.mt_idx[g];
    if (act) P.mt_idx[(size_t)(1 + slot) * G + g] = packed;
    int generated = 0;
    if (NP > 0) {
      MtChunkStream r;
      r.open(P.mt, act ? (uint32_t)g * 624u : 0u, packed, (uint8_t *)lds_raw + SK_TILE * SK_DECK_STRIDE, lane);
      STAMP(2);
      deal_compact<NP>(P, lds_raw, lane, r, ep, dst, act);
      if (act) P.mt_idx[g] = r.close();
      generated = r.chunks_made * 16;
    } else if (act) {
      uint8_t *fp = (uint8_t *)lds_raw + P.L.chunks * 1024 + lane * 4;
      MtStream<64> r;
      r.open(P.mt + (size_t)g * 624, packed, fp);
      r.stp = &st;
      STAMP(2);
      deal_into_lds(P, lp, r, ep);
      P.mt_idx[g] = r.close();
      generated = r.wp - (((16 - ((packed >> 16) & 15)) & 15) + (packed >> 16));
    }
    if (act) {
      uint32_t *mt = P.mt + (size_t)g * 624;
      mt_overrun = generated > 624 - 64;
      if (mt_overrun) {
        int k0 = (packed & 0xffff) + (packed >> 16);
        k0 = k0 >= 624 ? k0 - 624 : k0;
        int k1 = k0 + generated;
        k1 = k1 >= 624 ? k1 - 624 : k1;
        mt_untwist(mt, k0, k1);
        P.mt_idx[g] = packed;
      }
      STAMP(3);
    }
  } else if (act) {
    if (NP > 0) {
      PhiloxChunkStream r;
      r.open(P.seeds[g] + 1, ep, 0u, 0u);
      deal_compact<NP>(P, lds_raw, lane, r, ep, dst, true);
    } else {
      PhiloxStream r;
      r.open(P.seeds[g] + 1, ep, 0u, 0u);
      deal_into_lds(P, lp, r, ep);
    }
  }
  if (act) {
    if (NP == 0) store_spare(P, lp, slot, g);
    STAMP(4);
  }
  if (publish_inline == 1 || publish_inline == 2) {
    if (act) {
      if (!mt_overrun) P.spare_ready[(size_t)slot * G + g] = 1;
      P.busy[g] = 0;
    }
  } else {
    SK_FENCE_RELEASE(P);
    if (act)
      __hip_atomic_store(&P.done_flag[g], P.deal_tag | (mt_overrun ? 0x80000000u : 0u), __ATOMIC_RELAXED,
                         __HIP_MEMORY_SCOPE_AGENT);
  }
#ifdef SK_STAMPS
  if (lane == 0 && tile < P.tiles)
    for (int k = 0; k < 8; k++) P.stamps[(size_t)(P.tiles + tile) * 8 + k] += st.acc[k];
#endif
  TRACE_STORE(1, P.deal_tag, lane, block);
}

template <int NP>
__global__ __launch_bounds__(SK_TILE) void k_deal(SkParams P, int list_sel, int publish_inline) {
  extern __shared__ uint32_t lds_raw[];
  deal_body<NP>(P, list_sel, publish_inline, (int)blockIdx.x, (int)threadIdx.x, lds_raw);
}
```

### skyjo_rl_amd/csrc/skyjo_device.h

```cpp
#pragma once
#include <hip/hip_runtime.h>
#include <stdint.h>

#include "../../include/skyjo_vec.h"
#include "skyjo_layout.h"
#include "skyjo_draw.h"

struct SkCounters {
  unsigned long long steps, episodes, illegal, resets, sum_len, reshuffles, iters, waits;
  double sum_score[SKYJO_MAX_PLAYERS];
  double sum_reward[SKYJO_MAX_PLAYERS];
  double sum_reward_sq[SKYJO_MAX_PLAYERS];
  double sum_refunded[SKYJO_MAX_PLAYERS];
};
#define SK_ERR_DEAL_TIMEOUT 1u
#ifndef SK_SCORE_EVERY
#define SK_SCORE_EVERY 32
#endif
#define SK_ACC_KINDS 4

#ifndef SK_BANK
#define SK_BANK 3
#endif

struct SkParams {
  SkLayout L;
  int32_t B, tiles, rng_mode, auto_reset;
  uint32_t deal_tag;
  uint32_t spin_log2;
  uint32_t debug_deal_delay;
  double score_penalty, mean_reward, reward_refunded, illegal_reward;
  uint64_t game_id0;
  uint4 *state;
  uint4 *spare;
  uint8_t *spare_ready;
  uint8_t *bank_head;
  uint8_t *busy;
  uint8_t *cancel;
  uint32_t *done_flag;
  uint32_t *plan_tag;
  uint32_t *plan_ep;
  uint32_t ov_flags;
  uint32_t plan_new_tag;
  uint32_t be_add, be_read;
  uint32_t wg_local;
  uint32_t host_seq;
  int32_t *deal_list;
  uint32_t *deal_ep;
  uint32_t *deal_count;
  uint32_t *bank_empty;
  volatile uint32_t *health_host;
  uint32_t *mt;
  int32_t *mt_idx;
  uint64_t *seeds;
  uint32_t *deals_consumed;
  double *rewards;
  double *scores;
  uint8_t *done;
  double *acc_tile;
  uint32_t *dev_error;
  SkCounters *counters;
  unsigned long long *tile_counters;
  unsigned long long *stamps;
};

struct LaneCounters {
  uint32_t steps = 0, episodes = 0, illegal = 0, resets = 0, sum_len = 0, reshuffles = 0, waits = 0;
};

#define SK_FENCE_ACQUIRE(P)                                              \
  do {                                                                   \
    if ((P).wg_local) __builtin_amdgcn_fence(__ATOMIC_ACQUIRE, "workgroup"); \
    else __builtin_amdgcn_fence(__ATOMIC_ACQUIRE, "agent");              \
  } while (0)
#define SK_FENCE_RELEASE(P)                                              \
  do {                                                                   \
    if ((P).wg_local) __builtin_amdgcn_fence(__ATOMIC_RELEASE, "workgroup"); \
    else __builtin_amdgcn_fence(__ATOMIC_RELEASE, "agent");              \
  } while (0)
#define SK_RARE(x) __builtin_expect(!!(x), 0)
#define SK_OFTEN(x) __builtin_expect(!!(x), 1)
#define LIDX(b) ((((b) >> 4) << 10) | ((b) & 15))
#define LB(b) (lp[LIDX(b)])
#define LI(b) ((int)(int8_t)lp[LIDX(b)])
#define LW(w) (*(uint32_t *)(lp + LIDX(4 * (w))))
#define LH(b) (*(uint16_t *)(lp + LIDX(b)))
#define LSH(b) (*(int16_t *)(lp + LIDX(b)))
#define LQ(c) (*(uint4 *)(lp + ((c) << 10)))

__device__ __forceinline__ void tile_load(const SkParams &P, const uint4 *src, int tile, int lane, uint8_t *lp) {
  const uint4 *s = src + (size_t)tile * P.L.chunks * SK_TILE + lane;
  const int n = P.L.chunks;
  for (int c = 0; c < n; c += 6) {
    uint4 v[6];
#pragma unroll
    for (int k = 0; k < 6; k++)
      if (c + k < n) v[k] = s[(size_t)(c + k) * SK_TILE];
#pragma unroll
    for (int k = 0; k < 6; k++)
      if (c + k < n) LQ(c + k) = v[k];
  }
}

__device__ __forceinline__ void tile_store(const SkParams &P, uint4 *dst, int tile, int lane, uint8_t *lp) {
  uint4 *d = dst + (size_t)tile * P.L.chunks * SK_TILE + lane;
  const int n = P.L.chunks;
  for (int c = 0; c < n; c += 6) {
    uint4 v[6];
#pragma unroll
    for (int k = 0; k < 6; k++)
      if (c + k < n) v[k] = LQ(c + k);
#pragma unroll
    for (int k = 0; k < 6; k++)
      if (c + k < n) d[(size_t)(c + k) * SK_TILE] = v[k];
  }
}

typedef uint32_t sk_u32x4_nt __attribute__((ext_vector_type(4)));
__device__ __forceinline__ void tile_store_nt(const SkParams &P, uint4 *dst, int tile, int lane, uint8_t *lp) {
  sk_u32x4_nt *d = (sk_u32x4_nt *)(dst + (size_t)tile * P.L.chunks * SK_TILE + lane);
  const int n = P.L.chunks;
  for (int c = 0; c < n; c += 6) {
    uint4 v[6];
#pragma unroll
    for (int k = 0; k < 6; k++)
      if (c + k < n) v[k] = LQ(c + k);
#pragma unroll
    for (int k = 0; k < 6; k++)
      if (c + k < n) __builtin_nontemporal_store((sk_u32x4_nt){v[k].x, v[k].y, v[k].z, v[k].w}, d + (size_t)(c + k) * SK_TILE);
  }
}

#define SK_DMA4(NT)                                                                                                     \
  asm volatile("s_mov_b32 %0, m0\n\ts_mov_b32 m0, %3\n\ts_nop 0\n\t"                                                    \
               "global_load_lds_dwordx4 %1, %2" NT "\n\tglobal_load_lds_dwordx4 %1, %2 offset:1024" NT "\n\t"           \
               "global_load_lds_dwordx4 %1, %2 offset:2048" NT "\n\tglobal_load_lds_dwordx4 %1, %2 offset:3072" NT "\n\t" \
               "s_mov_b32 m0, %0"                                                                                       \
               : "=&s"(keep)                                                                                            \
               : "v"(voff), "s"(base), "s"(lds)                                                                         \
               : "memory")
#define SK_DMA1(NT)                                                                                              \
  asm volatile("s_mov_b32 %0, m0\n\ts_mov_b32 m0, %3\n\ts_nop 0\n\tglobal_load_lds_dwordx4 %1, %2" NT "\n\ts_mov_b32 m0, %0" \
               : "=&s"(keep)                                                                                     \
               : "v"(voff), "s"(base), "s"(lds)                                                                  \
               : "memory")
template <bool NT>
__device__ __forceinline__ void dma_record(const uint8_t *base, uint32_t voff, uint32_t lds, int chunks) {
  uint32_t keep;
  int c = 0;
  for (; c + 4 <= chunks; c += 4) {
    if (NT) SK_DMA4(" nt");
// ... 99 lines not shown
```

### skyjo_rl_amd/csrc/skyjo_layout.h

```cpp
#pragma once
#include <stdint.h>

#define SK_TILE 64
#define SK_NCARDS 150

#define H_PHASE 0
#define H_PLAYER 1
#define H_FLAGS 2
#define H_STATUS 3
#define H_NDRAW 4
#define H_NDISC 5
#define H_ROLE 6
#define H_TOP 7
#define H_EPLEN 8
#define H_RESH 10
#define H_HAND 11
#define H_EPISODE 12
#define H_MINSUM 16
#define H_MINHID 17
#define H_HIST 18
#define H_FINISHER 33
#define H_BANK 34
#define H_END 36
#define H_PILE H_END
#define PB_CARDS 0
#define PB_SUM 12
#define PB_HIDDEN 14
#define PB_REFUNDED 15
#define PB_VIS 16
#define PB_PLACED 28
#define PB_BYTES 32

#define F_TERMINATED 1
#define F_DONE 2
#define F_VALID 4

struct SkLayout {
  int32_t N, indirect, D, Dp, rec_bytes;
  int32_t off_pile, off_players;
  int32_t state_bytes, chunks;
};

#ifdef __HIPCC__
#define SK_HD __host__ __device__
#else
#define SK_HD
#endif
SK_HD static inline SkLayout sk_make_layout(int N, int indirect) {
  SkLayout L;
  L.N = N;
  L.indirect = indirect ? 1 : 0;
  L.D = indirect ? 31 : 19 + 12 * N;
  L.Dp = (L.D + 3) & ~3;
  L.rec_bytes = (L.Dp + 32 + 15) & ~15;
  L.off_pile = H_PILE;
  L.off_players = (H_PILE + SK_NCARDS + 15) & ~15;
  L.state_bytes = L.off_players + PB_BYTES * N;
  L.chunks = L.state_bytes / 16;
  return L;
}
SK_HD static inline int sk_pb(const SkLayout &L, int p) { return L.off_players + PB_BYTES * p; }
```

### skyjo_rl_amd/csrc/skyjo_record.h

```cpp
#pragma once
#ifndef SKYJO_DEVICE_PARTS
#error "include skyjo_device.h"
#endif

template <bool INDIRECT>
__device__ __forceinline__ void emit_record(const SkParams &P, uint8_t *lp, const HdrRegs &h, const ObsRegs &ob, int action,
                                            uint8_t *out, uint4 *held = nullptr, const uint4 *pre_a = nullptr, uint32_t pre_b = 0) {
  const int phase = h.w0 & 0xff;
  const uint32_t q0 = ob.q0, q1 = ob.q1, q2 = ob.q2;
  const uint32_t act24 = ((uint32_t)action & 0xffu) << 24;
  uint32_t m[8];
  {
    const uint32_t pm = phase ? 0xffffffffu : 0u;
    m[0] = ob.nz0 & pm, m[1] = ob.nz1 & pm, m[2] = ob.nz2 & pm, m[3] = ob.hd0 & pm, m[4] = ob.hd1 & pm, m[5] = ob.hd2 & pm;
    m[6] = (phase ? 0u : 0x0101u) | (((h.w0 >> 8) & 0xffu) << 16) | ((uint32_t)phase << 24);
    m[7] = (((h.w0 >> 16) & F_DONE) ? 1u : 0u) | ((h.w0 >> 24) << 8) | ((h.w2 & 0xffffu) << 16);
  }
  const uint4 a = pre_a ? *pre_a : LQ(1);
  const uint32_t s8 = (pre_a ? pre_b : (uint32_t)LB(32)) | ((h.w1 >> 24) << 8) | ((h.w2 >> 24) << 16);
  if (INDIRECT) {
    uint4 *o = (uint4 *)out;
    uint4 b;
    b.x = s8 | (q0 << 24), b.y = (q0 >> 8) | (q1 << 24), b.z = (q1 >> 8) | (q2 << 24), b.w = (q2 >> 8) | act24;
    if (held) {
      held[0] = a, held[1] = b, held[2] = make_uint4(m[0], m[1], m[2], m[3]), held[3] = make_uint4(m[4], m[5], m[6], m[7]);
    } else {
      o[0] = a, o[1] = b;
      o[2] = make_uint4(m[0], m[1], m[2], m[3]);
      o[3] = make_uint4(m[4], m[5], m[6], m[7]);
    }
  } else {
    uint32_t *o = (uint32_t *)out;
    const int N = P.L.N;
    o[0] = a.x, o[1] = a.y, o[2] = a.z, o[3] = a.w;
    uint32_t carry = s8;
    for (int p = 0; p < N; p++) {
      const uint4 r = LQ((sk_pb(P.L, p) + PB_VIS) >> 4);
      o[4 + 3 * p] = carry | (r.x << 24);
      o[5 + 3 * p] = (r.x >> 8) | (r.y << 24);
      o[6 + 3 * p] = (r.y >> 8) | (r.z << 24);
      carry = r.z >> 8;
    }
    o[4 + 3 * N] = carry | act24;
    uint32_t *om = o + (P.L.Dp >> 2);
#pragma unroll
    for (int w = 0; w < 8; w++) om[w] = m[w];
  }
}

__device__ __forceinline__ size_t bank_rec16(const SkParams &P, int slot, int g) {
  return ((size_t)slot * P.tiles * SK_TILE + (size_t)g) * P.L.chunks;
}
__device__ __forceinline__ void load_spare(const SkParams &P, uint8_t *lp, int slot, int tile, int lane) {
  const uint4 *s = P.spare + bank_rec16(P, slot, tile * SK_TILE + lane);
  const int n = P.L.chunks;
  for (int c = 0; c < n; c += 6) {
    uint4 v[6];
#pragma unroll
    for (int k = 0; k < 6; k++)
      if (c + k < n) v[k] = s[c + k];
#pragma unroll
    for (int k = 0; k < 6; k++)
      if (c + k < n) LQ(c + k) = v[k];
  }
}
__device__ __forceinline__ void store_spare(const SkParams &P, uint8_t *lp, int slot, int g) {
  uint4 *d = P.spare + bank_rec16(P, slot, g);
  const int n = P.L.chunks;
  for (int c = 0; c < n; c += 6) {
    uint4 v[6];
#pragma unroll
    for (int k = 0; k < 6; k++)
      if (c + k < n) v[k] = LQ(c + k);
#pragma unroll
    for (int k = 0; k < 6; k++)
      if (c + k < n) d[c + k] = v[k];
  }
}

__device__ __forceinline__ void bank_advance(const SkParams &P, uint8_t *lp, int g, int head, uint32_t dc) {
  const uint8_t nh = (uint8_t)((head + 1) % SK_BANK);
  P.bank_head[g] = nh;
  LB(H_BANK) = nh;
  P.deals_consumed[g] = dc + 1;
  P.done[g] = 0;
}

__device__ __forceinline__ bool consume_spare(const SkParams &P, uint8_t *lp, int tile, int lane, int g, int head) {
  const size_t G = (size_t)P.tiles * SK_TILE;
  const uint8_t ready = P.spare_ready[(size_t)head * G + g];
  const uint32_t dc = P.deals_consumed[g];
  if (!ready) return false;
  load_spare(P, lp, head, tile, lane);
  P.spare_ready[(size_t)head * G + g] = 0;
  bank_advance(P, lp, g, head, dc);
  return true;
}

struct SpareRegs {
  uint32_t dc;
  int head;
  uint8_t ready;
};
__device__ __forceinline__ void spare_issue(const SkParams &P, uint8_t *lp, uint32_t lds_tile, int tile, int lane, int g, SpareRegs &r) {
  const size_t G = (size_t)P.tiles * SK_TILE;
  r.head = LB(H_BANK) % SK_BANK;
  r.ready = P.spare_ready[(size_t)r.head * G + g];
  r.dc = P.deals_consumed[g];
  const uint32_t voff = (uint32_t)(bank_rec16(P, r.head, g) * 16);
  asm volatile("s_waitcnt lgkmcnt(0)" ::: "memory");
  dma_bank_record<false>((const uint8_t *)P.spare, voff, lds_tile, P.L.chunks);
}
__device__ __forceinline__ bool spare_commit(const SkParams &P, uint8_t *lp, int g, const SpareRegs &r) {
  sk_vm_drain();
  if (!r.ready) return false;
  P.spare_ready[(size_t)r.head * (size_t)P.tiles * SK_TILE + g] = 0;
  bank_advance(P, lp, g, r.head, r.dc);
  return true;
}

__device__ __forceinline__ constexpr int sk_stage_stride(int rec_bytes) { return ((rec_bytes >> 2) & 7) == 0 ? rec_bytes + 16 : rec_bytes; }

__device__ __forceinline__ bool deal_inline(const SkParams &P, uint8_t *lp, uint8_t *fp, int g, int tile, int lane, int head);
```

### skyjo_rl_amd/csrc/skyjo_step.h

```cpp
#pragma once
#ifndef SKYJO_DEVICE_PARTS
#error "include skyjo_device.h"
#endif

__device__ __forceinline__ void sk_publish_deals(const SkParams &P, int g) {
  const size_t G = (size_t)P.tiles * SK_TILE;
  const int b = P.busy[g];
  if (b) {
    const uint32_t tag = P.plan_tag[g];
    const uint32_t f = __hip_atomic_load(&P.done_flag[g], __ATOMIC_RELAXED, __HIP_MEMORY_SCOPE_AGENT);
    if ((f & 0x7fffffffu) == tag) {
      SK_FENCE_ACQUIRE(P);
      if (!P.cancel[g] && f == tag) P.spare_ready[(size_t)(b - 1) * G + g] = 1;
      P.busy[g] = 0, P.cancel[g] = 0;
    }
  }
}
__device__ __forceinline__ void sk_plan_deals(const SkParams &P, int g, int lane) {
  const size_t G = (size_t)P.tiles * SK_TILE;
  bool need = false, empty = false;
  if (g < P.B) {
    const uint8_t busy = P.busy[g];
    const int head = P.bank_head[g] % SK_BANK;
    const uint32_t consumed = P.deals_consumed[g];
    uint8_t ready[SK_BANK];
#pragma unroll
    for (int k = 0; k < SK_BANK; k++) ready[k] = P.spare_ready[(size_t)k * G + g];
    bool open = true;
    int r = 0;
#pragma unroll
    for (int k = 0; k < SK_BANK; k++) {
      uint8_t f = 0;
#pragma unroll
      for (int j = 0; j < SK_BANK; j++) f = (head + k) % SK_BANK == j ? ready[j] : f;
      open = open && f != 0;
      r += open ? 1 : 0;
    }
    need = !busy && r < SK_BANK;
    empty = need && r == 0;
    if (need) {
      P.busy[g] = (uint8_t)(1 + (head + r) % SK_BANK);
      P.cancel[g] = 0;
      P.plan_ep[g] = consumed + (uint32_t)r;
      P.plan_tag[g] = P.plan_new_tag;
    }
  }
  const unsigned long long be = __ballot(empty);
  if (be && lane == 0) atomicAdd(P.bank_empty + (P.be_add & 1u), (uint32_t)__popcll(be));
}

__device__ __forceinline__ void sk_error_to_host(const SkParams &P, int lane) {
  if (lane == 0) {
    const uint32_t e = __hip_atomic_load(P.dev_error, __ATOMIC_RELAXED, __HIP_MEMORY_SCOPE_AGENT);
    if (e) P.health_host[2] = e;
  }
}
__device__ __forceinline__ void sk_export_raw(const SkParams &P, uint8_t *lp, int g, uint8_t *o) {
  for (int c = 0; c < P.L.chunks; c++) ((uint4 *)o)[c] = LQ(c);
  double *d = (double *)(o + P.L.state_bytes);
  for (int p = 0; p < P.L.N; p++) d[p] = P.rewards[(size_t)g * P.L.N + p], d[P.L.N + p] = P.scores[(size_t)g * P.L.N + p];
  uint32_t *m = (uint32_t *)(d + 2 * P.L.N);
  m[0] = P.rng_mode == SKYJO_RNG_MT19937 ? (uint32_t)P.mt_idx[g] : 0u;
  m[1] = P.done[g];
}

__device__ __forceinline__ uint32_t sk_next_tag(uint32_t t) {
  t = (t + 1u) & 0x7fffffffu;
  return t ? t : 1u;
}
template <bool INDIRECT, bool POLICY, int NP, bool PLANAR = false>
__device__ __forceinline__ void step_body(const SkParams &Pin, const int tile, const int lane, uint32_t *lds_raw, const int32_t *actions,
                                          uint8_t *rec_out, int32_t *act_out, int iters, uint64_t policy_seed, uint64_t iter0,
                                          double *end_rew_out, uint8_t *end_out, uint8_t *raw_out, int raw_stride, const int cycle_len = 0,
                                          const bool defer_ok = true) {
  SkParams P = Pin;
  TRACE_DECL;
  if (NP > 0) P.L = sk_make_layout(NP, INDIRECT ? 1 : 0);
  const int g = tile * SK_TILE + lane;
  const uint32_t lds_tile = (uint32_t)(uintptr_t)(__attribute__((address_space(3))) uint32_t *)lds_raw;
  uint8_t *lp = (uint8_t *)lds_raw + lane * 16;
  uint8_t *stg = (uint8_t *)lds_raw + P.L.chunks * 1024;
  uint8_t *fp = stg + lane * 4;
  const int stg_bytes = (INDIRECT || PLANAR) ? 4096 : SK_TILE * (P.L.rec_bytes + 16);
  uint8_t *ap = stg + stg_bytes + lane * 8;
  constexpr bool DEFER = POLICY && NP > 0 && NP < 8;
  constexpr bool REGACC = NP > 0 && NP < 8;
  constexpr int NACC = REGACC ? SK_ACC_KINDS * NP : 1;
  double racc_store[NACC];
#pragma unroll
  for (int k = 0; k < NACC; k++) racc_store[k] = 0.0;
  double *racc = REGACC ? racc_store : nullptr;
  uint8_t *pendp = DEFER && defer_ok ? stg + stg_bytes + (REGACC ? 0 : SK_ACC_KINDS * P.L.N * 512) + lane * 16 : nullptr;
  int pend_fin = -1;
  if (!REGACC)
    for (int k = 0; k < SK_ACC_KINDS * P.L.N; k++) ACC(k) = 0.0;
  STAMP_DECL;
  if (!POLICY) tile_load(P, P.state, tile, lane, lp);
  else dma_record<true>((const uint8_t *)P.state, (uint32_t)((((size_t)tile * P.L.chunks) * SK_TILE + lane) * 16), lds_tile, P.L.chunks);
  if (P.ov_flags & 1u) sk_publish_deals(P, g);
  sk_vm_drain();
  HdrRegs h;
  HDR_LOAD(h);
  STAMP(0);
  const bool valid = ((h.w0 >> 16) & F_VALID) != 0;
  LaneCounters cnt;
  uint32_t r0 = 0, r1 = 0, r2 = 0, r3 = 0;
  const uint64_t gid = P.game_id0 + (uint64_t)g;
  ObsRegs ob;
  if (valid) obs_load(P, lp, (h.w0 >> 8) & 0xff, ob);
  for (int it = 0; it < iters; it++) {
    const uint64_t iter = iter0 + (uint64_t)it;
    if (POLICY && (it == 0 || (iter & 3) == 0)) {
      philox4x32_10((uint32_t)(iter >> 2), (uint32_t)gid, (uint32_t)(gid >> 32), 0x504F4C00u, (uint32_t)policy_seed,
                    (uint32_t)(policy_seed >> 32), r0, r1, r2, r3);
      for (int k = (int)(iter & 3); k > 0; k--) {
        const uint32_t t = r0;
        r0 = r1, r1 = r2, r2 = r3, r3 = t;
      }
    }
    STAMP_T(3);
    const uint32_t word = r0;
    if (POLICY) {
      r0 = r1, r1 = r2, r2 = r3, r3 = word;
    }
    int a = -1;
    if (valid) {
      const bool over = ((h.w0 >> 16) & F_DONE) != 0;
      if (!POLICY) a = actions[g];
      const bool skip = !POLICY && a == SKYJO_ACTION_SKIP;
      const bool acted = !over && !skip;
      SpareRegs sp;
      const bool resetting = over && P.auto_reset && !skip;
      if (resetting) spare_issue(P, lp, lds_tile, tile, lane, g, sp);
      STAMP_T(4);
      if (!over && !skip) {
        const uint32_t v0 = ob.q0, v1 = ob.q1, v2 = ob.q2;
        STAMP_N(2);
        const uint4 row_pre = LQ(sk_pb(P.L, (h.w0 >> 8) & 0xff) >> 4);
        asm volatile("" ::: "memory");
        if (POLICY) a = policy_pick(h.w0 & 0xff, ob, word);
#ifndef SK_STAMPS_FINE
        STAMP_N(3);
#endif
        apply_action<INDIRECT, NP, POLICY>(P, lp, fp, ap, h, v0, v1, v2, a, g, cnt, st, pendp, pend_fin, row_pre, racc);
#ifdef SK_STAMPS_FINE
        STAMP(6);
#else
        STAMP(5);
#endif
      } else if (!skip) {
        a = -1;
        if (P.auto_reset) {
          bool dealt = true;
          if (!spare_commit(P, lp, g, sp)) {
            dealt = deal_inline(P, lp, fp, g, tile, lane, sp.head);
            cnt.waits++;
          }
          HDR_LOAD(h);
          if (SK_OFTEN(dealt)) {
            h.w0 = (h.w0 & 0x00ffffffu) | ((uint32_t)SKYJO_ST_RESET << 24);
            cnt.resets++;
          }
        } else {
          h.w0 = (h.w0 & 0x00ffffffu) | ((uint32_t)SKYJO_ST_NOOP_DONE << 24);
        }
        STAMP(1);
      } else {
        a = -1;
      }
      if (!POLICY && acted && (unsigned)a >= (unsigned)SKYJO_NUM_ACTIONS) a = -2;
      if (!POLICY && end_out) {
        const bool end = acted && ((h.w0 >> 16) & F_DONE) != 0;
        end_out[g] = end ? 1 : 0;
        for (int q = 0; q < P.L.N; q++) end_rew_out[(size_t)g * P.L.N + q] = end ? P.rewards[(size_t)g * P.L.N + q] : 0.0;
      }
      const uint4 rec_a = LQ(1);
      const uint32_t rec_b = LB(32);
      const uint4 rec_row = LQ((sk_pb(P.L, (h.w0 >> 8) & 0xff) + PB_VIS) >> 4);
      asm volatile("" ::: "memory");
      obs_from_row(rec_row, ob);
      if (rec_out) {
        if (INDIRECT) {
// ... 10 lines not shown
          }
        } else if (PLANAR) {
          constexpr int PIECES = NP > 0 ? (((19 + 12 * NP + 3) & ~3) + 32 + 15) / 16 : 1;
          uint32_t wbuf[4 * PIECES];
#pragma unroll
          for (int k = 0; k < 4 * PIECES; k++) wbuf[k] = 0u;
          emit_record<INDIRECT>(P, lp, h, ob, a, (uint8_t *)wbuf, nullptr, &rec_a, rec_b);
          typedef uint32_t u32x4_t __attribute__((ext_vector_type(4)));
          uint8_t *blk = rec_out + ((size_t)it * P.tiles + (size_t)tile) * (SK_TILE * 16 * PIECES) + lane * 16;
#pragma unroll
          for (int p = 0; p < PIECES; p++)
            __builtin_nontemporal_store((u32x4_t){wbuf[4 * p], wbuf[4 * p + 1], wbuf[4 * p + 2], wbuf[4 * p + 3]}, (u32x4_t *)(blk + p * 1024));
        } else {
          emit_record<INDIRECT>(P, lp, h, ob, a, stg + lane * sk_stage_stride(P.L.rec_bytes), nullptr, &rec_a, rec_b);
        }
      }
      if (act_out) __builtin_nontemporal_store(a, &act_out[(size_t)it * P.B + g]);
#ifdef SK_STAMPS_FINE
      STAMP(7);
#else
      STAMP(6);
#endif
    }
    if (DEFER && ((it & (SK_SCORE_EVERY - 1)) == SK_SCORE_EVERY - 1 || it == iters - 1)) {
      if (SK_RARE(__any(pend_fin >= 0))) {
        if (pend_fin >= 0) {
          finish_game_fixed<(NP > 0 && NP < 8) ? NP : 1>(P, pendp, 1024, ap, g, pend_fin, racc);
          pend_fin = -1;
        }
      }
    }
    if (!INDIRECT && !PLANAR && rec_out) {
      typedef uint32_t u32x4_t __attribute__((ext_vector_type(4)));
      const int pieces = P.L.rec_bytes >> 4, stride = sk_stage_stride(P.L.rec_bytes);
      uint8_t *blk = rec_out + ((size_t)it * P.B + (size_t)tile * SK_TILE) * (size_t)P.L.rec_bytes;
      const int live = P.B - tile * SK_TILE;
      for (int q0 = lane; q0 < pieces * SK_TILE; q0 += 4 * SK_TILE) {
        uint4 v[4];
#pragma unroll
        for (int j = 0; j < 4; j++) {
          const int q = q0 + j * SK_TILE, r = q / pieces, p = q - r * pieces;
          if (q < pieces * SK_TILE) v[j] = *(const uint4 *)(stg + r * stride + p * 16);
        }
        if (SK_OFTEN(live >= SK_TILE)) {
#pragma unroll
          for (int j = 0; j < 4; j++) {
            const int q = q0 + j * SK_TILE;
            if (q0 - lane + j * SK_TILE < pieces * SK_TILE)
              __builtin_nontemporal_store((u32x4_t){v[j].x, v[j].y, v[j].z, v[j].w}, (u32x4_t *)(blk + (size_t)q * 16));
          }
        } else {
#pragma unroll
          for (int j = 0; j < 4; j++) {
            const int q = q0 + j * SK_TILE, r = q / pieces;
            if (q < pieces * SK_TILE && r < live)
              __builtin_nontemporal_store((u32x4_t){v[j].x, v[j].y, v[j].z, v[j].w}, (u32x4_t *)(blk + (size_t)q * 16));
          }
        }
      }
    }
    if (INDIRECT && !PLANAR && rec_out) {
      typedef uint32_t u32x4_t __attribute__((ext_vector_type(4)));
      uint8_t *blk = rec_out + ((size_t)it * P.B + (size_t)tile * SK_TILE) * 64;
      const int live = P.B - tile * SK_TILE;
      uint4 v[4];
#pragma unroll
      for (int j = 0; j < 4; j++) {
        const int r = 16 * j + (lane >> 2), p = lane & 3;
        v[j] = *(const uint4 *)(stg + r * 64 + ((p + (r >> 1)) & 3) * 16);
      }
      if (SK_OFTEN(live >= SK_TILE)) {
#pragma unroll
        for (int j = 0; j < 4; j++)
          __builtin_nontemporal_store((u32x4_t){v[j].x, v[j].y, v[j].z, v[j].w}, (u32x4_t *)(blk + j * 1024 + lane * 16));
      } else {
#pragma unroll
        for (int j = 0; j < 4; j++)
          if (16 * j + (lane >> 2) < live)
            __builtin_nontemporal_store((u32x4_t){v[j].x, v[j].y, v[j].z, v[j].w}, (u32x4_t *)(blk + j * 1024 + lane * 16));
      }
    }
    STAMP_T(2);
    if (POLICY && cycle_len && it + 1 < iters && (it + 1) % cycle_len == 0) {
      if (P.busy[g]) (void)wait_deal_done(P, g);
      sk_publish_deals(P, g);
      sk_plan_deals(P, g, lane);
      P.plan_new_tag = sk_next_tag(P.plan_new_tag);
      TRACE_WAIT_BEGIN;
      __syncthreads();
      TRACE_WAIT_END;
    }
  }
  HDR_FLUSH(h);
  tile_store_nt(P, P.state, tile, lane, lp);
  if (!POLICY && raw_out && valid) sk_export_raw(P, lp, g, raw_out + (size_t)g * raw_stride);
  if (P.ov_flags & 2u) {
    if (P.ov_flags & 1u) {
      if (P.busy[g]) (void)wait_deal_done(P, g);
      sk_publish_deals(P, g);
    }
    sk_plan_deals(P, g, lane);
  }
  if (!POLICY) {
    sk_error_to_host(P, lane);
    if (P.host_seq) {
      __threadfence_system();
      if (lane == 0) __hip_atomic_store(&P.health_host[3], P.host_seq, __ATOMIC_RELEASE, __HIP_MEMORY_SCOPE_SYSTEM);
    }
  }
  uint32_t v[7] = {cnt.steps, cnt.episodes, cnt.illegal, cnt.resets, cnt.sum_len, cnt.reshuffles, cnt.waits};
#pragma unroll
  for (int k = 0; k < 7; k++)
    for (int off = 32; off > 0; off >>= 1) v[k] += __shfl_down(v[k], off, 64);
  if (lane == 0) {
    unsigned long long *c = P.tile_counters + (size_t)tile * 8;
#pragma unroll
    for (int k = 0; k < 7; k++) c[k] += v[k];
  }
  if (__any(cnt.episodes | cnt.illegal)) {
    double mine = 0.0;
    if (REGACC) {
#pragma unroll
      for (int k = 0; k < NACC; k++) {
        double x = racc_store[k];
        for (int off = 32; off > 0; off >>= 1) x += __shfl_down(x, off, 64);
        x = __shfl(x, 0, 64);
        mine = lane == k ? x : mine;
      }
    } else {
      for (int k = 0; k < SK_ACC_KINDS * P.L.N; k++) {
        double x = ACC(k);
        for (int off = 32; off > 0; off >>= 1) x += __shfl_down(x, off, 64);
        x = __shfl(x, 0, 64);
        mine = lane == k ? x : mine;
      }
    }
    if (lane < SK_ACC_KINDS * P.L.N)
      P.acc_tile[(size_t)tile * SK_ACC_KINDS * SKYJO_MAX_PLAYERS + (lane / P.L.N) * SKYJO_MAX_PLAYERS + lane % P.L.N] += mine;
  }
  STAMP(7);
  STAMP_STORE;
  TRACE_STORE(0, (uint32_t)(iter0 / (uint64_t)(iters > 0 ? iters : 1)), lane, tile);
}

template <bool INDIRECT, bool POLICY, int NP, bool PLANAR = false>
__global__ __launch_bounds__(SK_TILE) void k_step(SkParams Pin, const int32_t *actions, uint8_t *rec_out,
                                                  int32_t *act_out, int iters, uint64_t policy_seed, uint64_t iter0,
                                                  double *end_rew_out, uint8_t *end_out, uint8_t *raw_out, int raw_stride) {
  extern __shared__ uint32_t lds_raw[];
  step_body<INDIRECT, POLICY, NP, PLANAR>(Pin, (int)blockIdx.x, (int)threadIdx.x, lds_raw, actions, rec_out, act_out, iters, policy_seed, iter0,
                                          end_rew_out, end_out, raw_out, raw_stride);
}

template <bool INDIRECT>
__device__ __forceinline__ void sk_emit_to(const SkParams &P, uint8_t *lp, const HdrRegs &h, const ObsRegs &ob, uint8_t *rec_out, int tile, int lane,
                                           int planar) {
  const int g = tile * SK_TILE + lane;
  if (INDIRECT && planar) {
    uint4 rr[4];
    emit_record<INDIRECT>(P, lp, h, ob, -1, nullptr, rr);
    uint4 *o = (uint4 *)(rec_out + (size_t)tile * SK_TILE * P.L.rec_bytes) + lane;
#pragma unroll
    for (int k = 0; k < 4; k++) o[k * SK_TILE] = rr[k];
  } else {
    emit_record<INDIRECT>(P, lp, h, ob, -1, rec_out + (size_t)g * P.L.rec_bytes);
  }
}

template <bool INDIRECT>
__global__ __launch_bounds__(SK_TILE) void k_observe(SkParams P, const int32_t *players, uint8_t *rec_out, int planar) {
  extern __shared__ uint32_t lds_raw[];
  const int tile = blockIdx.x, lane = threadIdx.x, g = tile * SK_TILE + lane;
  uint8_t *lp = (uint8_t *)lds_raw + lane * 16;
  sk_error_to_host(P, lane);
  tile_load(P, P.state, tile, lane, lp);
  if (!(LB(H_FLAGS) & F_VALID)) return;
  HdrRegs h;
  HDR_LOAD(h);
  int q = players ? players[g] : LB(H_PLAYER);
  q = q < 0 ? 0 : (q >= P.L.N ? P.L.N - 1 : q);
  ObsRegs ob;
  obs_load(P, lp, q, ob);
  sk_emit_to<INDIRECT>(P, lp, h, ob, rec_out, tile, lane, planar);
}

template <bool INDIRECT>
__global__ __launch_bounds__(SK_TILE) void k_reset(SkParams P, const uint8_t *mask, uint8_t *rec_out, uint8_t *raw_out, int raw_stride, int planar) {
  extern __shared__ uint32_t lds_raw[];
  const int tile = blockIdx.x, lane = threadIdx.x, g = tile * SK_TILE + lane;
  uint8_t *lp = (uint8_t *)lds_raw + lane * 16;
  uint8_t *fp = (uint8_t *)lds_raw + P.L.chunks * 1024 + lane * 4;
  if (g >= P.B) return;
  const bool want = !mask || mask[g];
  bool want_counted = false;
  tile_load(P, P.state, tile, lane, lp);
  if (want) {
    const int head = P.bank_head[g] % SK_BANK;
    bool dealt = true;
    if (!consume_spare(P, lp, tile, lane, g, head)) dealt = deal_inline(P, lp, fp, g, tile, lane, head);
    if (dealt) LB(H_STATUS) = SKYJO_ST_RESET;
    want_counted = dealt;
  }
  HdrRegs h;
  HDR_LOAD(h);
  if (rec_out) {
    ObsRegs ob;
    obs_load(P, lp, LB(H_PLAYER), ob);
    sk_emit_to<INDIRECT>(P, lp, h, ob, rec_out, tile, lane, planar);
  }
  if (want) tile_store(P, P.state, tile, lane, lp);
  if (raw_out && (LB(H_FLAGS) & F_VALID)) sk_export_raw(P, lp, g, raw_out + (size_t)g * raw_stride);
  sk_error_to_host(P, lane);
  const unsigned long long wb = __ballot(want_counted);
  if (want_counted && lane == __ffsll((long long)wb) - 1) P.tile_counters[(size_t)tile * 8 + 3] += __popcll(wb);
}
```

### skyjo_rl_amd/csrc/skyjo_transition.h

```cpp
#pragma once
#ifndef SKYJO_DEVICE_PARTS
#error "include skyjo_device.h"
#endif

__device__ __forceinline__ void refresh_minima(const SkParams &P, uint8_t *lp) {
  int ms = LSH(sk_pb(P.L, 0) + PB_SUM), mh = LB(sk_pb(P.L, 0) + PB_HIDDEN);
  for (int q = 1; q < P.L.N; q++) {
    int s = LSH(sk_pb(P.L, q) + PB_SUM), h = LB(sk_pb(P.L, q) + PB_HIDDEN);
    ms = s < ms ? s : ms, mh = h < mh ? h : mh;
  }
  LB(H_MINSUM) = (uint8_t)(int8_t)(ms < 127 ? ms : 127);
  LB(H_MINHID) = (uint8_t)mh;
}

template <class Rng>
__device__ __forceinline__ void reshuffle_discard(const SkParams &P, uint8_t *lp, Rng &r) {
  const int n = LB(H_NDISC), role = LB(H_ROLE), pb = P.L.off_pile;
  const int reg = role ? 0 : 1;
  for (int i = n - 1; i >= 1; i--) {
    int j = (int)rng_interval(r, (uint32_t)i);
    int ai = pb + pile_addr(reg, i), aj = pb + pile_addr(reg, j);
    uint8_t t = LB(ai);
    LB(ai) = LB(aj), LB(aj) = t;
  }
  for (int k = 0; k < n - 1; k++) LB(H_HIST + 2 + LI(pb + pile_addr(reg, k)))--;
  int last = LI(pb + pile_addr(reg, n - 1));
  LB(pb + pile_addr(reg ^ 1, 0)) = (uint8_t)last;
  LB(H_NDRAW) = (uint8_t)(n - 1), LB(H_NDISC) = 1, LB(H_ROLE) = (uint8_t)(role ^ 1);
  LB(H_TOP) = (uint8_t)last;
  int rs = LB(H_RESH);
  LB(H_RESH) = (uint8_t)(rs < 255 ? rs + 1 : 255);
}

#define SK_WAIT_OK 0
#define SK_WAIT_GAVE_UP 1
#define SK_WAIT_TIMEOUT 2
__device__ __forceinline__ int wait_deal_done(const SkParams &P, int g) {
  uint32_t f = 0;
  const uint32_t tag = P.plan_tag[g];
  for (int spin = 0; spin < (1 << P.spin_log2); spin++) {
    f = __hip_atomic_load(&P.done_flag[g], __ATOMIC_RELAXED, __HIP_MEMORY_SCOPE_AGENT);
    if ((f & 0x7fffffffu) == tag) break;
    __builtin_amdgcn_s_sleep(32);
  }
  if ((f & 0x7fffffffu) != tag) {
    atomicOr(P.dev_error, SK_ERR_DEAL_TIMEOUT);
    return SK_WAIT_TIMEOUT;
  }
  SK_FENCE_ACQUIRE(P);
  return (f >> 31) != 0 ? SK_WAIT_GAVE_UP : SK_WAIT_OK;
}

__device__ __forceinline__ uint32_t mt_untwist_y(const uint32_t *mt, int i) {
  uint32_t t = mt[i] ^ mt[i + 397 >= 624 ? i + 397 - 624 : i + 397];
  const uint32_t odd = t >> 31;
  t ^= odd ? 0x9908b0dfu : 0u;
  return (t << 1) | odd;
}
__device__ __forceinline__ void mt_untwist(uint32_t *mt, int from, int to) {
  for (int i = to; i != from;) {
    const int nx = i == 624 ? 0 : i;
    i = nx == 0 ? 623 : nx - 1;
    const uint32_t y = mt_untwist_y(mt, i);
    const int ip1 = i == 623 ? 0 : i + 1;
    mt[ip1] = (mt[ip1] & 0x80000000u) | (y & 0x7fffffffu);
    mt[i] = y & 0x80000000u;
  }
}

__device__ __forceinline__ int mt_rollback(const SkParams &P, uint32_t *mt, int g, int slot, int packed) {
  const size_t G = (size_t)P.tiles * SK_TILE;
  const int snap = P.mt_idx[(size_t)(1 + slot) * G + g];
  int from = (snap & 0xffff) + (snap >> 16), to = (packed & 0xffff) + (packed >> 16);
  from = from >= 624 ? from - 624 : from, to = to >= 624 ? to - 624 : to;
  mt_untwist(mt, from, to);
  return snap;
}

__device__ __forceinline__ void reshuffle_dispatch(const SkParams &P, uint8_t *lp, uint8_t *fp, int g) {
  if (P.rng_mode == SKYJO_RNG_MT19937) {
    const size_t G = (size_t)P.tiles * SK_TILE;
    uint32_t *mt = P.mt + (size_t)g * 624;
    const int head = LB(H_BANK) % SK_BANK;
    const int busy = P.busy[g];
    const bool inflight = busy && !P.cancel[g];
    bool undo_inflight = false;
    if (inflight) {
      const int w = wait_deal_done(P, g);
      if (w == SK_WAIT_TIMEOUT) {
        LB(H_FLAGS) |= F_DONE, LB(H_STATUS) = SKYJO_ST_ERROR, LB(H_NDRAW) = 1;
        P.done[g] = 1;
        for (int q = 0; q < P.L.N; q++) P.rewards[(size_t)g * P.L.N + q] = 0.0;
        return;
      }
      undo_inflight = w == SK_WAIT_OK;
      P.cancel[g] = 1;
    }
    int packed = P.mt_idx[g];
    if (undo_inflight) packed = mt_rollback(P, mt, g, busy - 1, packed);
    for (int k = SK_BANK - 1; k >= 0; k--) {
      const int slot = (head + k) % SK_BANK;
      if (P.spare_ready[(size_t)slot * G + g]) {
        packed = mt_rollback(P, mt, g, slot, packed);
        P.spare_ready[(size_t)slot * G + g] = 0;
      }
    }
    MtStream<16> r;
    r.open(mt, packed, fp);
    reshuffle_discard(P, lp, r);
    P.mt_idx[g] = r.close();
  } else {
    PhiloxStream r;
    r.open(P.seeds[g] + 1, *(uint32_t *)(lp + LIDX(H_EPISODE)), LB(H_RESH), 1u);
    reshuffle_discard(P, lp, r);
  }
}

#define ACC(k) (*(double *)(ap + ((k) << 9)))
__device__ __forceinline__ void acc_add(uint8_t *ap, int k, double v) {
  __hip_atomic_fetch_add(&ACC(k), v, __ATOMIC_RELAXED, __HIP_MEMORY_SCOPE_WAVEFRONT);
}
__device__ __forceinline__ void acc_episode(uint8_t *ap, int N, int p, double score, double reward, int refunded) {
  acc_add(ap, p, score), acc_add(ap, N + p, reward), acc_add(ap, 2 * N + p, reward * reward);
  if (refunded) acc_add(ap, 3 * N + p, (double)refunded);
}

__device__ __forceinline__ void finish_game(const SkParams &P, uint8_t *lp, uint8_t *fp, uint8_t *ap, int g,
                                            int finisher) {
  const int N = P.L.N;
  double *sc = P.scores + (size_t)g * N, *rw = P.rewards + (size_t)g * N;
  int mn = 0, fs = 0;
  for (int p = 0; p < N; p++) {
    int s = 0;
    for (int c = 0; c < 4; c++) {
      int b = sk_pb(P.L, p) + PB_CARDS + 3 * c;
      int t0 = LI(b), t1 = LI(b + 1), t2 = LI(b + 2);
      if (!(t0 == t1 && t1 == t2)) s += t0 + t1 + t2;
    }
    MT_FIFO(p) = (uint32_t)s;
    mn = (p == 0 || s < mn) ? s : mn;
    fs = p == finisher ? s : fs;
  }
  const bool penal = mn != fs;
#define SCORE(p) ((penal && (p) == finisher) ? (double)(int)MT_FIFO(p) * P.score_penalty : (double)(int)MT_FIFO(p))
  double sum;
  if (N < 8) {
    sum = 0.0;
    for (int p = 0; p < N; p++) sum += SCORE(p);
  } else {
    sum = ((SCORE(0) + SCORE(1)) + (SCORE(2) + SCORE(3))) + ((SCORE(4) + SCORE(5)) + (SCORE(6) + SCORE(7)));
    for (int p = 8; p < N; p++) sum += SCORE(p);
  }
  const double mean = sum / (double)N;
  for (int p = 0; p < N; p++) {
    const double d = SCORE(p);
    double r = (-d + mean) + P.mean_reward;
    const int rf = LB(sk_pb(P.L, p) + PB_REFUNDED);
    if (P.reward_refunded != 0.0) r += (double)rf * P.reward_refunded;
    sc[p] = d, rw[p] = r;
    acc_episode(ap, N, p, d, r, rf);
  }
#undef SCORE
  P.done[g] = 1;
}

template <int NP>
__device__ __forceinline__ void finish_game_fixed(const SkParams &P, const uint8_t *rows, int stride, uint8_t *ap, int g, int finisher,
                                                  double *racc = nullptr) {
  double *sc = P.scores + (size_t)g * NP, *rw = P.rewards + (size_t)g * NP;
  int s[NP], refunded[NP];
  int mn = 0, fs = 0;
#pragma unroll
  for (int p = 0; p < NP; p++) {
    const uint4 row = *(const uint4 *)(rows + p * stride);
    const uint32_t c0 = row.x, c1 = row.y, c2 = row.z;
    refunded[p] = (int)(row.w >> 24);
    const uint32_t tri[4] = {c0 & 0xffffffu, (c0 >> 24) | ((c1 & 0xffffu) << 8), (c1 >> 16) | ((c2 & 0xffu) << 16), c2 >> 8};
    int t = 0;
#pragma unroll
    for (int c = 0; c < 4; c++) {
      const int t0 = (int)(int8_t)tri[c], t1 = (int)(int8_t)(tri[c] >> 8), t2 = (int)(int8_t)(tri[c] >> 16);
      t += (t0 == t1 && t1 == t2) ? 0 : t0 + t1 + t2;
    }
    s[p] = t;
    mn = (p == 0 || t < mn) ? t : mn;
    fs = p == finisher ? t : fs;
  }
  const bool penal = mn != fs;
  double d[NP], sum = 0.0;
#pragma unroll
  for (int p = 0; p < NP; p++) {
    d[p] = (penal && p == finisher) ? (double)s[p] * P.score_penalty : (double)s[p];
    sum += d[p];
  }
  const double mean = sum / (double)NP;
#pragma unroll
  for (int p = 0; p < NP; p++) {
    double r = (-d[p] + mean) + P.mean_reward;
    if (P.reward_refunded != 0.0) r += (double)refunded[p] * P.reward_refunded;
    sc[p] = d[p], rw[p] = r;
    if (racc) {
      racc[p] += d[p], racc[NP + p] += r, racc[2 * NP + p] += r * r, racc[3 * NP + p] += (double)refunded[p];
    } else {
      acc_episode(ap, NP, p, d[p], r, refunded[p]);
    }
  }
}

struct HdrRegs {
  uint32_t w0, w1, w2;
};
#define HDR_LOAD(h) ((h).w0 = LW(0), (h).w1 = LW(1), (h).w2 = LW(2))
#define HDR_FLUSH(h) (LW(0) = (h).w0, LW(1) = (h).w1, LW(2) = (h).w2)

__device__ __forceinline__ int byte3(uint32_t a, uint32_t b, uint32_t c, int k) {
  const uint32_t w = k < 4 ? a : (k < 8 ? b : c);
  return (int)(int8_t)(w >> ((k & 3) * 8));
}
__device__ __forceinline__ void put3(uint32_t &a, uint32_t &b, uint32_t &c, int k, int val) {
  const uint32_t sh = (uint32_t)(k & 3) * 8u, m = ~(0xffu << sh), v = ((uint32_t)val & 0xffu) << sh;
  if (k < 4) a = (a & m) | v;
  else if (k < 8) b = (b & m) | v;
  else c = (c & m) | v;
}
__device__ __forceinline__ void hist_add(uint8_t *lp, int value, int delta) {
  const int b = H_HIST + 2 + value;
  uint32_t *w = (uint32_t *)(lp + LIDX(b & ~3));
  const uint32_t d = (uint32_t)delta << ((b & 3) * 8);
  __hip_atomic_fetch_add(w, d, __ATOMIC_RELAXED, __HIP_MEMORY_SCOPE_WAVEFRONT);
}
__device__ __forceinline__ uint32_t swar_nonzero01(uint32_t x) {
  return ((((x & 0x7f7f7f7fu) + 0x7f7f7f7fu) | x) & 0x80808080u) >> 7;
}
__device__ __forceinline__ uint32_t pack12(uint32_t a, uint32_t b, uint32_t c) {
  return ((a * 0x00204081u >> 21) & 0xfu) | (((b * 0x00204081u >> 21) & 0xfu) << 4) |
         (((c * 0x00204081u >> 21) & 0xfu) << 8);
}

struct ObsRegs {
  uint32_t q0, q1, q2, nz0, nz1, nz2, hd0, hd1, hd2;
};
__device__ __forceinline__ void obs_from_row(const uint4 &row, ObsRegs &o) {
  o.q0 = row.x, o.q1 = row.y, o.q2 = row.z;
  o.nz0 = swar_nonzero01(o.q0 ^ 0xf2f2f2f2u);
  o.nz1 = swar_nonzero01(o.q1 ^ 0xf2f2f2f2u);
  o.nz2 = swar_nonzero01(o.q2 ^ 0xf2f2f2f2u);
  o.hd0 = swar_nonzero01(o.q0 ^ 0x0f0f0f0fu) ^ 0x01010101u;
  o.hd1 = swar_nonzero01(o.q1 ^ 0x0f0f0f0fu) ^ 0x01010101u;
  o.hd2 = swar_nonzero01(o.q2 ^ 0x0f0f0f0fu) ^ 0x01010101u;
}
__device__ __forceinline__ void obs_load(const SkParams &P, uint8_t *lp, int q, ObsRegs &o) {
  const uint4 row = LQ((sk_pb(P.L, q) + PB_VIS) >> 4);
  obs_from_row(row, o);
}

__device__ __forceinline__ int policy_pick(int phase, const ObsRegs &o, uint32_t word) {
  if (phase == 0) return 24 + (int)__umulhi(word, 2u);
  uint32_t legal = pack12(o.nz0, o.nz1, o.nz2) | (pack12(o.hd0, o.hd1, o.hd2) << 12);
  const int n = __popc(legal);
  if (n == 0) return 24;
  int k = (int)__umulhi(word, (uint32_t)n), pos = 0;
  int c = __popc(legal & 0xfffu);
  if (k >= c) k -= c, pos = 12, legal >>= 12;
  c = __popc(legal & 0x3fu);
  if (k >= c) k -= c, pos += 6, legal >>= 6;
  c = __popc(legal & 0x7u);
  if (k >= c) k -= c, pos += 3, legal >>= 3;
  c = (int)(legal & 1u);
  if (k >= c) {
    k -= c, pos += 1;
    c = (int)((legal >> 1) & 1u);
    if (k >= c) pos += 1;
  }
  return pos;
}

template <bool INDIRECT, int NP, bool TRUSTED>
__device__ __forceinline__ void apply_action(const SkParams &P, uint8_t *lp, uint8_t *fp, uint8_t *ap, HdrRegs &h, uint32_t v0,
                                             uint32_t v1, uint32_t v2, int a, int g, LaneCounters &cnt, Stamps &st,
                                             uint8_t *pendp, int &pend_fin, const uint4 &row_pre, double *racc = nullptr) {
  const int N = P.L.N;
  const int phase = h.w0 & 0xff, p = (h.w0 >> 8) & 0xff;
  const int blk = sk_pb(P.L, p), cardb = blk + PB_CARDS, visb = blk + PB_VIS, pb = P.L.off_pile;
  const unsigned ua = (unsigned)a;
  int slot = 0, sv = 0;
  bool legal;
  if (ua < 24u) {
    slot = a < 12 ? a : a - 12;
    sv = byte3(v0, v1, v2, slot);
    legal = phase == 1 && (TRUSTED || (a < 12 ? sv != SKYJO_REFUNDED : sv == SKYJO_HAND_NONE));
  } else {
    legal = (TRUSTED || ua <= 25u) && phase == 0;
  }
  if (!legal) {
    double *rw = P.rewards + (size_t)g * N;
    for (int q = 0; q < N; q++) rw[q] = q == p ? P.illegal_reward : 0.0;
    if (NP > 0 && racc) {
#pragma unroll
      for (int q = 0; q < (NP > 0 ? NP : 1); q++)
        racc[NP + q] += q == p ? P.illegal_reward : 0.0, racc[2 * NP + q] += q == p ? P.illegal_reward * P.illegal_reward : 0.0;
    } else {
      acc_add(ap, N + p, P.illegal_reward), acc_add(ap, 2 * N + p, P.illegal_reward * P.illegal_reward);
    }
    h.w0 = (h.w0 & 0x0000ffffu) | ((((h.w0 >> 16) & 0xffu) | F_DONE) << 16) | ((uint32_t)SKYJO_ST_ILLEGAL << 24);
    P.done[g] = 1;
    cnt.illegal++;
    return;
  }
  const int eplen = (int)(h.w2 & 0xffffu) + 1;
  h.w2 = (h.w2 & 0xffff0000u) | (uint32_t)eplen;
  h.w0 &= 0x00ffffffu;
  cnt.steps++;
  if (phase == 0) {
    const int role = (h.w1 >> 16) & 1;
    int nd = h.w1 & 0xff;
    const int ns = (h.w1 >> 8) & 0xff;
    const int hidden_p = (int)((row_pre.w >> 16) & 0xffu);
    int pile_top = LI(pb + pile_addr(role, nd > 0 ? nd - 1 : 0));
    const int disc_top = LI(pb + pile_addr(role ^ 1, ns > 0 ? ns - 1 : 0));
    const int disc_below = LI(pb + pile_addr(role ^ 1, ns > 1 ? ns - 2 : 0));

    if (hidden_p == 0) {
      h.w0 |= (uint32_t)(F_TERMINATED | F_DONE) << 16;
      LB(H_FINISHER) = (uint8_t)p;
      if (NP > 0 && NP < 8) {
        constexpr int NQ = (NP > 0 && NP < 8) ? NP : 1;
        P.done[g] = 1;
        if (pendp) {
#pragma unroll
          for (int q = 0; q < NQ; q++) *(uint4 *)(pendp + q * 1024) = LQ(sk_pb(P.L, q) >> 4);
          pend_fin = p;
        } else {
          finish_game_fixed<NQ>(P, lp + (P.L.off_players >> 4) * 1024, 2048, ap, g, p, racc);
        }
      } else {
        finish_game(P, lp, fp, ap, g, p);
      }
      cnt.episodes++;
      cnt.sum_len += eplen;
#ifdef SK_STAMPS_FINE
      STAMP(3);
#endif
      return;
    }
    const bool from_pile = a == 24;
    if (from_pile && nd == 0) {
      HDR_FLUSH(h);
      reshuffle_dispatch(P, lp, fp, g);
      HDR_LOAD(h);
      cnt.reshuffles++;
      nd = h.w1 & 0xff;
      pile_top = LI(pb + pile_addr((h.w1 >> 16) & 1, nd - 1));
    }
    int hand;
    if (from_pile) {
      hand = pile_top;
      h.w1 = (h.w1 & 0xffffff00u) | (uint32_t)(nd - 1);
    } else {
      hand = disc_top;
      hist_add(lp, hand, -1);
      const int top = ns > 1 ? disc_below : -3;
      h.w1 = (h.w1 & 0x00ff00ffu) | ((uint32_t)(ns - 1) << 8) | (((uint32_t)top & 0xffu) << 24);
    }
    h.w2 = (h.w2 & 0x00ffffffu) | (((uint32_t)hand & 0xffu) << 24);
    h.w0 = (h.w0 & 0xffffff00u) | 1u;
#ifdef SK_STAMPS_FINE
    STAMP(3);
#endif
    return;
  }
  STAMP_N(4);
  const int hand = (int)(int8_t)(h.w2 >> 24);
  const int reg = ((h.w1 >> 16) & 1) ^ 1;
  int ns = (h.w1 >> 8) & 0xff;
  const uint4 row = row_pre;
  const uint32_t c0 = row.x, c1 = row.y, c2 = row.z;
  int sum = (int)(int16_t)(row.w & 0xffffu), hid = (int)((row.w >> 16) & 0xffu), refunded = (int)(row.w >> 24);
  int oms = 1 << 20, omh = 1 << 20;
  for (int q = 0; q < N; q++) {
    const uint32_t cq = LW((sk_pb(P.L, q) + PB_SUM) >> 2);
    const int s = (int)(int16_t)(cq & 0xffffu), hq = (int)((cq >> 16) & 0xffu);
    oms = (q != p && s < oms) ? s : oms, omh = (q != p && hq < omh) ? hq : omh;
  }
#ifdef SK_STAMPS_FINE
  STAMP(5);
#endif
  const bool swap = a < 12, was_hidden = sv == SKYJO_HAND_NONE;
  const int under = byte3(c0, c1, c2, slot);
  const int shown = swap ? hand : under, gone = swap ? under : hand;
  LB(pb + pile_addr(reg, ns)) = (uint8_t)gone;
  ns++;
  hist_add(lp, gone, 1);
  LB(cardb + slot) = (uint8_t)shown;
  LB(visb + slot) = (uint8_t)shown;
  put3(v0, v1, v2, slot, shown);
  sum += shown - (was_hidden ? 0 : under);
  hid -= was_hidden ? 1 : 0;
  if (!INDIRECT) {
    if (!was_hidden) hist_add(lp, under, -1);
    hist_add(lp, shown, 1);
  }
  int top = gone;
  {
    const uint32_t tri[4] = {v0 & 0xffffffu, (v0 >> 24) | ((v1 & 0xffffu) << 8), (v1 >> 16) | ((v2 & 0xffu) << 16), v2 >> 8};
    bool full[4];
#pragma unroll
    for (int c = 0; c < 4; c++) {
      const uint32_t b0 = tri[c] & 0xffu;
      full[c] = ((tri[c] ^ (tri[c] >> 8)) & 0xffffu) == 0 && b0 != (uint32_t)SKYJO_HAND_NONE && b0 != ((uint32_t)SKYJO_REFUNDED & 0xffu);
    }
// ... 30 lines not shown
```

Baseline: 48.02 billion.

## Pack per-game deal-bank bookkeeping into one 16-byte record

Replaces the separate per-game arrays (spare_ready per slot, bank_head, busy, cancel, plan_tag, plan_ep, deals_consumed, done) with a single uint4 bank record per game, loaded and stored as one vector access. The step, deal and publish paths now do one 16-byte load and at most one store instead of many scattered byte and word accesses. Snapshot/restore and the done-pointer API gain conversion kernels that pack and unpack the old field layout, and done_ptr now launches a kernel and synchronises on every call. Concurrent writers to different fields of the same record (the step kernel and the overlapped dealing kernel) could now overwrite each other's updates.

```diff
diff --git a/skyjo_rl_amd/csrc/skyjo_capi.hip b/skyjo_rl_amd/csrc/skyjo_capi.hip
--- a/skyjo_rl_amd/csrc/skyjo_capi.hip
+++ b/skyjo_rl_amd/csrc/skyjo_capi.hip
@@ -150,7 +150,13 @@
   uint8_t *d_mask = nullptr;
   void *sel_scratch = nullptr;
   size_t sel_blocks = 0;
-  std::vector<std::pair<void *, size_t>> allocs;
+  struct Alloc {
+    void *first;
+    size_t second;
+    int field;
+  };
+  std::vector<Alloc> allocs;
+  uint8_t *d_done = nullptr;
   std::vector<void *> owned;
   uint8_t *arena = nullptr;
   size_t arena_off = 0;
@@ -189,8 +195,39 @@
   return dev_error_check(h);
 }
 
+enum BankField { BF_READY, BF_HEAD, BF_BUSY, BF_CANCEL, BF_PLAN_TAG, BF_PLAN_EP, BF_CONSUMED, BF_DONE, BF_COUNT };
+struct BankFields {
+  uint8_t *p[BF_COUNT];
+};
+__global__ __launch_bounds__(256) void k_bank_fields(uint4 *bank, BankFields f, int G, int pack) {
+  const int g = blockIdx.x * blockDim.x + threadIdx.x;
+  if (g >= G) return;
+  if (pack) {
+    uint4 r;
+    uint32_t ready = f.p[BF_CANCEL][g] ? BK_CANCEL_BIT : 0u;
+    for (int k = 0; k < SK_BANK; k++) ready |= f.p[BF_READY][(size_t)k * G + g] ? BK_READY_BIT(k) : 0u;
+    r.x = (uint32_t)f.p[BF_HEAD][g] | ready | (uint32_t)f.p[BF_BUSY][g] << 16 | (uint32_t)(f.p[BF_DONE][g] != 0) << 24;
+    r.y = ((const uint32_t *)f.p[BF_CONSUMED])[g], r.z = ((const uint32_t *)f.p[BF_PLAN_EP])[g], r.w = ((const uint32_t *)f.p[BF_PLAN_TAG])[g];
+    bank[g] = r;
+  } else {
+    const uint4 r = bank[g];
+    for (int k = 0; k < SK_BANK; k++) f.p[BF_READY][(size_t)k * G + g] = BK_READY(r, k) ? 1 : 0;
+    f.p[BF_HEAD][g] = (uint8_t)BK_HEAD(r), f.p[BF_BUSY][g] = (uint8_t)BK_BUSY(r), f.p[BF_CANCEL][g] = BK_CANCEL(r) ? 1 : 0;
+    f.p[BF_DONE][g] = (uint8_t)BK_DONE(r);
+    ((uint32_t *)f.p[BF_CONSUMED])[g] = r.y, ((uint32_t *)f.p[BF_PLAN_EP])[g] = r.z, ((uint32_t *)f.p[BF_PLAN_TAG])[g] = r.w;
+  }
+}
+__global__ __launch_bounds__(256) void k_bank_done(const uint4 *bank, uint8_t *done, int G) {
+  const int g = blockIdx.x * blockDim.x + threadIdx.x;
+  if (g < G) done[g] = (uint8_t)BK_DONE(bank[g]);
+}
+
+void bank_field(skyjo_vec *h, int field, size_t bytes) {
+  if (h->arena_mode != 1) h->allocs.push_back({nullptr, bytes, field});
+}
+
 template <class T>
-int dalloc(skyjo_vec *h, T **out, size_t count, bool zero = true) {
+int dalloc(skyjo_vec *h, T **out, size_t count, bool zero = true, bool in_snapshot = true) {
   const size_t bytes = count * sizeof(T);
   void *p = nullptr;
   if (h->arena_mode) {
@@ -207,7 +244,7 @@
     h->owned.push_back(p);
   }
   if (zero) HIPCHK(hipMemset(p, 0, bytes));
-  h->allocs.emplace_back(p, bytes);
+  if (in_snapshot) h->allocs.push_back({p, bytes, -1});
   *out = (T *)p;
   return SKYJO_OK;
 }
@@ -553,15 +590,19 @@
     if (cfg->rng_mode == SKYJO_RNG_MT19937 && (rc = dalloc(h, &P.mt, h->G * 624 + 16, false)  )) {
       return rc;
     }
-    if ((rc = dalloc(h, &P.state, rec16)) || (rc = dalloc(h, &P.spare, SK_BANK * rec16)) ||
-        (rc = dalloc(h, &P.spare_ready, SK_BANK * h->G)) || (rc = dalloc(h, &P.bank_head, h->G)) ||
-        (rc = dalloc(h, &P.busy, h->G)) || (rc = dalloc(h, &P.cancel, h->G)) || (rc = dalloc(h, &P.done_flag, h->G)) || (rc = dalloc(h, &P.plan_tag, h->G)) || (rc = dalloc(h, &P.plan_ep, h->G)) ||
-        (rc = dalloc(h, &P.deal_list, 2 * h->G)) || (rc = dalloc(h, &P.deal_ep, 2 * h->G)) ||
+    if ((rc = dalloc(h, &P.state, rec16)) || (rc = dalloc(h, &P.spare, SK_BANK * rec16)) || (rc = dalloc(h, &P.bank, h->G, true, false))) return rc;
+    bank_field(h, BF_READY, SK_BANK * h->G), bank_field(h, BF_HEAD, h->G), bank_field(h, BF_BUSY, h->G), bank_field(h, BF_CANCEL, h->G);
+    if ((rc = dalloc(h, &P.done_flag, h->G))) return rc;
+    bank_field(h, BF_PLAN_TAG, 4 * h->G), bank_field(h, BF_PLAN_EP, 4 * h->G);
+    if ((rc = dalloc(h, &P.deal_list, 2 * h->G)) || (rc = dalloc(h, &P.deal_ep, 2 * h->G)) ||
         (rc = dalloc(h, &P.deal_count, 2)) || (rc = dalloc(h, &P.bank_empty, 2)) ||
-        (rc = dalloc(h, &P.mt_idx, (1 + SK_BANK) * h->G)) || (rc = dalloc(h, &P.seeds, h->G)) ||
-        (rc = dalloc(h, &P.deals_consumed, h->G)) || (rc = dalloc(h, &P.rewards, h->G * N)) ||
-        (rc = dalloc(h, &P.scores, h->G * N)) || (rc = dalloc(h, &P.done, h->G)) ||
-        (rc = dalloc(h, &P.acc_tile, (size_t)P.tiles * SK_ACC_KINDS * SKYJO_MAX_PLAYERS)) || (rc = dalloc(h, &P.dev_error, 1)) ||
+        (rc = dalloc(h, &P.mt_idx, (1 + SK_BANK) * h->G)) || (rc = dalloc(h, &P.seeds, h->G))) {
+      return rc;
+    }
+    bank_field(h, BF_CONSUMED, 4 * h->G);
+    if ((rc = dalloc(h, &P.rewards, h->G * N)) || (rc = dalloc(h, &P.scores, h->G * N))) return rc;
+    bank_field(h, BF_DONE, h->G);
+    if ((rc = dalloc(h, &P.acc_tile, (size_t)P.tiles * SK_ACC_KINDS * SKYJO_MAX_PLAYERS)) || (rc = dalloc(h, &P.dev_error, 1)) ||
         (rc = dalloc(h, &P.counters, 1)) || (rc = dalloc(h, &P.tile_counters, (size_t)P.tiles * 8)) || (rc = dalloc(h, &P.stamps, (size_t)P.tiles * 32))) {
       return rc;
     }
@@ -668,7 +709,6 @@
     HIPCHK(hipMemcpyAsync(d_seeds, seeds_host, sizeof(uint64_t) * (size_t)h->P.B, hipMemcpyHostToDevice, s));
   }
   HIPCHK(hipDeviceSynchronize());
-  HIPCHK(hipMemsetAsync(h->P.done, 0, h->G, s));
   HIPCHK(hipMemsetAsync(h->P.dev_error, 0, sizeof(uint32_t), s));
   h->health_host[2] = 0;
   int rc0;
@@ -735,8 +775,11 @@
     return fail(SKYJO_E_DEVICE, "hipMalloc failed for the snapshot");
   }
   size_t off = 0;
+  BankFields bf{};
   for (auto &a : h->allocs) {
-    hipError_t e = hipMemcpyAsync((uint8_t *)sn->blob + off, a.first, a.second, hipMemcpyDeviceToDevice, s);
+    hipError_t e = hipSuccess;
+    if (a.field >= 0) bf.p[a.field] = (uint8_t *)sn->blob + off;
+    else e = hipMemcpyAsync((uint8_t *)sn->blob + off, a.first, a.second, hipMemcpyDeviceToDevice, s);
     if (e != hipSuccess) {
       (void)hipFree(sn->blob);
       delete sn;
@@ -744,6 +787,7 @@
     }
     off += (a.second + 255) & ~(size_t)255;
   }
+  hipLaunchKernelGGL(k_bank_fields, dim3((unsigned)((h->G + 255) / 256)), dim3(256), 0, s, h->P.bank, bf, (int)h->G, 0);
   if (hipError_t e = hipStreamSynchronize(s); e != hipSuccess) {
     (void)hipFree(sn->blob);
     delete sn;
@@ -770,11 +814,15 @@
   if ((rc = publish_deals(h, s))) return rc;
   HIPCHK(hipDeviceSynchronize());
   size_t off = 0;
+  BankFields bf{};
   for (size_t k = 0; k < sn->array_bytes.size(); k++) {
     const auto &a = h->allocs[k];
-    HIPCHK(hipMemcpyAsync(a.first, (const uint8_t *)sn->blob + off, a.second, hipMemcpyDeviceToDevice, s));
+    if (a.field >= 0) bf.p[a.field] = (uint8_t *)sn->blob + off;
+    else HIPCHK(hipMemcpyAsync(a.first, (const uint8_t *)sn->blob + off, a.second, hipMemcpyDeviceToDevice, s));
     off += (a.second + 255) & ~(size_t)255;
   }
+  hipLaunchKernelGGL(k_bank_fields, dim3((unsigned)((h->G + 255) / 256)), dim3(256), 0, s, h->P.bank, bf, (int)h->G, 1);
+  HIPCHK(hipGetLastError());
   HIPCHK(hipStreamSynchronize(s));
   h->pending_iters = sn->pending_iters, h->deal_every_iters = sn->deal_every_iters, h->calm_runs = sn->calm_runs;
   h->list_sel = sn->list_sel, h->auto_interval = sn->auto_interval, h->health_seen = sn->health_seen;
@@ -972,7 +1020,22 @@
 
 const double *skyjo_vec_rewards_ptr(const skyjo_vec *h) { return h ? h->P.rewards : nullptr; }
 const double *skyjo_vec_scores_ptr(const skyjo_vec *h) { return h ? h->P.scores : nullptr; }
-const uint8_t *skyjo_vec_done_ptr(const skyjo_vec *h) { return h ? h->P.done : nullptr; }
+static int dense_done(skyjo_vec *h) {
+  if (!h->d_done) {
+    HIPCHK(hipMalloc((void **)&h->d_done, h->G));
+    h->owned.push_back(h->d_done);
+  }
+  hipLaunchKernelGGL(k_bank_done, dim3((unsigned)((h->G + 255) / 256)), dim3(256), 0, nullptr, h->P.bank, h->d_done, (int)h->G);
+  HIPCHK(hipGetLastError());
+  HIPCHK(hipStreamSynchronize(nullptr));
+  return SKYJO_OK;
+}
+const uint8_t *skyjo_vec_done_ptr(const skyjo_vec *h) {
+  if (!h) return nullptr;
+  skyjo_vec *m = const_cast<skyjo_vec *>(h);
+  GUARD(m);
+  return dense_done(m) == SKYJO_OK ? m->d_done : nullptr;
+}
 
 int skyjo_vec_sample_actions_layout(skyjo_vec *h, const void *records, int32_t layout, const float *logits, int64_t n, uint64_t seed,
                                     uint64_t ticket, int32_t no_masking, int32_t *actions_out, float *logp_out,
@@ -1408,12 +1471,12 @@
   r[H_MINHID] = (uint8_t)mh;
   r[H_TOP] = in->n_disc ? (uint8_t)in->discard_pile[in->n_disc - 1] : (uint8_t)(int8_t)-3;
   r[H_HAND] = (uint8_t)in->hand_card;
-  HIPCHK(hipMemcpyAsync(&r[H_BANK], h->P.bank_head + game, 1, hipMemcpyDeviceToHost, s));
+  HIPCHK(hipMemcpyAsync(&r[H_BANK], (const uint8_t *)(h->P.bank + game) + offsetof(SkBankRec, head), 1, hipMemcpyDeviceToHost, s));
   HIPCHK(hipStreamSynchronize(s));
   uint8_t *dst = (uint8_t *)(h->P.state + ((size_t)(game / SK_TILE) * L.chunks) * SK_TILE + game % SK_TILE);
   HIPCHK(hipMemcpy2DAsync(dst, SK_TILE * 16, r.data(), 16, 16, L.chunks, hipMemcpyHostToDevice, s));
   uint8_t dn = (r[H_FLAGS] & F_DONE) ? 1 : 0;
-  HIPCHK(hipMemcpyAsync(h->P.done + game, &dn, 1, hipMemcpyHostToDevice, s));
+  HIPCHK(hipMemcpyAsync((uint8_t *)(h->P.bank + game) + offsetof(SkBankRec, done), &dn, 1, hipMemcpyHostToDevice, s));
   if (dn) {
     HIPCHK(hipMemcpyAsync(h->P.rewards + (size_t)game * L.N, in->rewards, sizeof(double) * L.N, hipMemcpyHostToDevice, s));
     HIPCHK(hipMemcpyAsync(h->P.scores + (size_t)game * L.N, in->final_score, sizeof(double) * L.N,
@@ -1695,7 +1758,11 @@
   }
   if (rewards_out) HIPCHK(hipMemcpy(rewards_out, h->P.rewards, n * sizeof(double), hipMemcpyDeviceToHost));
   if (scores_out) HIPCHK(hipMemcpy(scores_out, h->P.scores, n * sizeof(double), hipMemcpyDeviceToHost));
-  if (done_out) HIPCHK(hipMemcpy(done_out, h->P.done, (size_t)h->P.B, hipMemcpyDeviceToHost));
+  if (done_out) {
+    int rc;
+    if ((rc = dense_done(h))) return rc;
+    HIPCHK(hipMemcpy(done_out, h->d_done, (size_t)h->P.B, hipMemcpyDeviceToHost));
+  }
   return dev_error_check(h);
 }
 
diff --git a/skyjo_rl_amd/csrc/skyjo_deal.h b/skyjo_rl_amd/csrc/skyjo_deal.h
--- a/skyjo_rl_amd/csrc/skyjo_deal.h
+++ b/skyjo_rl_amd/csrc/skyjo_deal.h
@@ -8,11 +8,9 @@
   if (i >= count) return;
   const int g = first + i;
   const uint64_t value = seeds ? seeds[i] : base + P.game_id0 + (uint64_t)g;
-  const size_t G = (size_t)P.tiles * SK_TILE;
   P.seeds[g] = value;
-  P.deals_consumed[g] = 0;
-  for (int k = 0; k < SK_BANK; k++) P.spare_ready[(size_t)k * G + g] = 0;
-  P.bank_head[g] = 0, P.busy[g] = 0, P.cancel[g] = 0, P.done_flag[g] = 0;
+  bank_store(P, g, make_uint4(0u, 0u, 0u, 0u));
+  P.done_flag[g] = 0;
   if (P.rng_mode == SKYJO_RNG_MT19937) {
     uint32_t *mt = P.mt + (size_t)g * 624;
     uint32_t x = (uint32_t)(value + 1);
@@ -35,8 +33,9 @@
     mt[k] = x;
   }
   P.mt_idx[g] = 0;
-  const size_t G = (size_t)P.tiles * SK_TILE;
-  for (int k = 0; k < SK_BANK; k++) P.spare_ready[(size_t)k * G + g] = 0;
+  uint4 bk = bank_load(P, g);
+  for (int k = 0; k < SK_BANK; k++) bk.x &= ~BK_READY_BIT(k);
+  bank_store(P, g, bk);
 }
 
 template <class Rng>
@@ -462,25 +461,27 @@
 }
 
 __device__ __forceinline__ bool deal_inline(const SkParams &P, uint8_t *lp, uint8_t *fp, int g, int tile, int lane, int head) {
-  const uint32_t ep = P.deals_consumed[g];
-  const int busy = P.busy[g];
+  uint4 bk = bank_load(P, g);
+  const uint32_t ep = bk.y;
+  const int busy = BK_BUSY(bk);
   if (busy) {
-    const bool cancelled = P.cancel[g] != 0;
+    const bool cancelled = BK_CANCEL(bk);
     if (P.rng_mode == SKYJO_RNG_MT19937 && !cancelled) {
-      const int w = wait_deal_done(P, g);
+      const int w = wait_deal_done(P, g, bk.w);
       if (w == SK_WAIT_TIMEOUT) {
         LB(H_FLAGS) = F_VALID | F_DONE, LB(H_STATUS) = SKYJO_ST_ERROR;
         for (int q = 0; q < P.L.N; q++) P.rewards[(size_t)g * P.L.N + q] = 0.0;
         return false;
       }
-      P.cancel[g] = 1;
       if (w == SK_WAIT_OK) {
         load_spare(P, lp, busy - 1, tile, lane);
-        bank_advance(P, lp, g, head, ep);
+        bk.x |= BK_CANCEL_BIT;
+        bank_advance(lp, head, bk);
+        bank_store(P, g, bk);
         return true;
       }
     }
-    P.cancel[g] = 1;
+    bk.x |= BK_CANCEL_BIT;
   }
   if (P.rng_mode == SKYJO_RNG_MT19937) {
     MtStream<16> r;
@@ -493,8 +494,9 @@
     deal_into_lds(P, lp, r, ep);
   }
   LB(H_BANK) = (uint8_t)head;
-  P.deals_consumed[g] = ep + 1;
-  P.done[g] = 0;
+  bk.y = ep + 1;
+  bk.x &= 0x00ffffffu;
+  bank_store(P, g, bk);
   return true;
 }
 
@@ -510,23 +512,13 @@
     bool need = false;
     int slot = 0, r = 0;
     uint32_t consumed = 0;
+    uint4 bk = make_uint4(0u, 0u, 0u, 0u);
     if (g < P.B) {
-      const uint8_t busy = P.busy[g];
-      const int head = P.bank_head[g] % SK_BANK;
-      consumed = P.deals_consumed[g];
-      uint8_t ready[SK_BANK];
-#pragma unroll
-      for (int k = 0; k < SK_BANK; k++) ready[k] = P.spare_ready[(size_t)k * G + g];
-      bool open = true;
-#pragma unroll
-      for (int k = 0; k < SK_BANK; k++) {
-        uint8_t f = 0;
-#pragma unroll
-        for (int j = 0; j < SK_BANK; j++) f = (head + k) % SK_BANK == j ? ready[j] : f;
-        open = open && f != 0;
-        r += open ? 1 : 0;
-      }
-      need = !busy && r < SK_BANK;
+      bk = bank_load(P, g);
+      const int head = BK_HEAD(bk) % SK_BANK;
+      consumed = bk.y;
+      r = bank_ready_run(bk);
+      need = !BK_BUSY(bk) && r < SK_BANK;
       slot = (head + r) % SK_BANK;
     }
     const unsigned long long b = __ballot(need);
@@ -550,9 +542,10 @@
       const uint32_t pos = block_first + wave_need[wave] + (uint32_t)__popcll(b & ((1ull << lane) - 1ull));
       list[pos] = g;
       eps[pos] = consumed + (uint32_t)r;
-      P.busy[g] = (uint8_t)(1 + slot);
-      P.cancel[g] = 0;
-      P.plan_tag[g] = P.deal_tag;
+      bank_set_busy(bk, 1 + slot);
+      bk.x &= ~BK_CANCEL_BIT;
+      bk.w = P.deal_tag;
+      bank_store(P, g, bk);
     }
     __syncthreads();
   }
@@ -569,15 +562,22 @@
   }
   for (int i = blockIdx.x * blockDim.x + threadIdx.x; i < count; i += gridDim.x * blockDim.x) {
     const int g = list[i];
-    const int slot = P.busy[g] - 1;
-    if (slot >= 0 && !P.cancel[g] && P.done_flag[g] == P.deal_tag) P.spare_ready[(size_t)slot * G + g] = 1;
-    P.busy[g] = 0, P.cancel[g] = 0;
+    uint4 bk = bank_load(P, g);
+    const int slot = BK_BUSY(bk) - 1;
+    if (slot >= 0 && !BK_CANCEL(bk) && P.done_flag[g] == P.deal_tag) bk.x |= BK_READY_BIT(slot);
+    bk.x &= ~(0x00ff0000u | BK_CANCEL_BIT);
+    bank_store(P, g, bk);
   }
 }
 
 __global__ __launch_bounds__(256) void k_publish_all(SkParams P) {
   const int g = blockIdx.x * blockDim.x + threadIdx.x;
-  if (g < P.tiles * SK_TILE) sk_publish_deals(P, g);
+  if (g < P.tiles * SK_TILE) {
+    const uint4 was = bank_load(P, g);
+    uint4 bk = was;
+    sk_publish_deals(P, g, bk);
+    sk_bank_put(P, g, bk, was);
+  }
 }
 
 template <int NP>
@@ -609,25 +609,15 @@
   int g, slot;
   uint32_t ep;
   bool act;
+  uint4 bk;
   if (fused) {
     const bool listed = i < P.B;
     g = listed ? i : 0;
-    const uint8_t busy = P.busy[g];
-    const int head = P.bank_head[g] % SK_BANK;
-    const uint32_t consumed = P.deals_consumed[g];
-    uint8_t ready[SK_BANK];
-#pragma unroll
-    for (int k = 0; k < SK_BANK; k++) ready[k] = P.spare_ready[(size_t)k * G + g];
-    bool open = true;
-    int r = 0;
-#pragma unroll
-    for (int k = 0; k < SK_BANK; k++) {
-      uint8_t f = 0;
-#pragma unroll
-      for (int j = 0; j < SK_BANK; j++) f = (head + k) % SK_BANK == j ? ready[j] : f;
-      open = open && f != 0;
-      r += open ? 1 : 0;
-    }
+    bk = bank_load(P, g);
+    const int busy = BK_BUSY(bk);
+    const int head = BK_HEAD(bk) % SK_BANK;
+    const uint32_t consumed = bk.y;
+    const int r = bank_ready_run(bk);
     act = listed && !busy && r < SK_BANK;
     slot = (head + r) % SK_BANK;
     ep = consumed + (uint32_t)r;
@@ -636,15 +626,17 @@
   } else if (piped) {
     const bool listed = i < P.B;
     g = listed ? i : 0;
-    const int owner = listed ? P.busy[g] : 0;
-    act = owner > 0 && P.plan_tag[g] == P.deal_tag;
+    bk = bank_load(P, g);
+    const int owner = listed ? BK_BUSY(bk) : 0;
+    act = owner > 0 && bk.w == P.deal_tag;
     slot = act ? owner - 1 : 0;
-    ep = P.plan_ep[g];
+    ep = bk.z;
   } else {
     const bool listed = i < count;
     g = listed ? P.deal_list[(size_t)list_sel * G + i] : 0;
     ep = listed ? P.deal_ep[(size_t)list_sel * G + i] : 0u;
-    const int owner = listed ? P.busy[g] : 0;
+    bk = bank_load(P, g);
+    const int owner = listed ? BK_BUSY(bk) : 0;
     act = owner > 0;
     slot = act ? owner - 1 : 0;
   }
@@ -701,8 +693,9 @@
   }
   if (publish_inline == 1 || publish_inline == 2) {
     if (act) {
-      if (!mt_overrun) P.spare_ready[(size_t)slot * G + g] = 1;
-      P.busy[g] = 0;
+      if (!mt_overrun) bk.x |= BK_READY_BIT(slot);
+      bank_set_busy(bk, 0);
+      bank_store(P, g, bk);
     }
   } else {
     SK_FENCE_RELEASE(P);
diff --git a/skyjo_rl_amd/csrc/skyjo_device.h b/skyjo_rl_amd/csrc/skyjo_device.h
--- a/skyjo_rl_amd/csrc/skyjo_device.h
+++ b/skyjo_rl_amd/csrc/skyjo_device.h
@@ -1,5 +1,6 @@
 #pragma once
 #include <hip/hip_runtime.h>
+#include <stddef.h>
 #include <stdint.h>
 
 #include "../../include/skyjo_vec.h"
@@ -33,13 +34,8 @@
   uint64_t game_id0;
   uint4 *state;
   uint4 *spare;
-  uint8_t *spare_ready;
-  uint8_t *bank_head;
-  uint8_t *busy;
-  uint8_t *cancel;
+  uint4 *bank;
   uint32_t *done_flag;
-  uint32_t *plan_tag;
-  uint32_t *plan_ep;
   uint32_t ov_flags;
   uint32_t plan_new_tag;
   uint32_t be_add, be_read;
@@ -53,10 +49,8 @@
   uint32_t *mt;
   int32_t *mt_idx;
   uint64_t *seeds;
-  uint32_t *deals_consumed;
   double *rewards;
   double *scores;
-  uint8_t *done;
   double *acc_tile;
   uint32_t *dev_error;
   SkCounters *counters;
@@ -67,6 +61,31 @@
 struct LaneCounters {
   uint32_t steps = 0, episodes = 0, illegal = 0, resets = 0, sum_len = 0, reshuffles = 0, waits = 0;
 };
+
+#define BK_HEAD(r) ((int)((r).x & 0xffu))
+#define BK_READY_BIT(slot) (0x100u << (slot))
+#define BK_READY(r, slot) (((r).x & BK_READY_BIT(slot)) != 0u)
+#define BK_CANCEL_BIT 0x8000u
+#define BK_CANCEL(r) (((r).x & BK_CANCEL_BIT) != 0u)
+#define BK_BUSY(r) ((int)(((r).x >> 16) & 0xffu))
+#define BK_DONE(r) ((int)((r).x >> 24))
+static_assert(SK_BANK <= 7, "the ready flags of a bank share one byte with the cancel bit");
+__device__ __forceinline__ uint4 bank_load(const SkParams &P, int g) { return P.bank[g]; }
+__device__ __forceinline__ void bank_store(const SkParams &P, int g, const uint4 &r) { P.bank[g] = r; }
+__device__ __forceinline__ void bank_set_busy(uint4 &r, int busy) { r.x = (r.x & 0xff00ffffu) | ((uint32_t)busy << 16); }
+__device__ __forceinline__ void bank_set_done(const SkParams &P, int g) { ((uint8_t *)(P.bank + g))[offsetof(SkBankRec, done)] = 1; }
+__device__ __forceinline__ uint8_t bank_get_done(const SkParams &P, int g) { return ((const uint8_t *)(P.bank + g))[offsetof(SkBankRec, done)]; }
+__device__ __forceinline__ int bank_ready_run(const uint4 &r) {
+  const int head = BK_HEAD(r) % SK_BANK;
+  bool open = true;
+  int n = 0;
+#pragma unroll
+  for (int k = 0; k < SK_BANK; k++) {
+    open = open && BK_READY(r, (head + k) % SK_BANK);
+    n += open ? 1 : 0;
+  }
+  return n;
+}
 
 #define SK_FENCE_ACQUIRE(P)                                              \
   do {                                                                   \
diff --git a/skyjo_rl_amd/csrc/skyjo_layout.h b/skyjo_rl_amd/csrc/skyjo_layout.h
--- a/skyjo_rl_amd/csrc/skyjo_layout.h
+++ b/skyjo_rl_amd/csrc/skyjo_layout.h
@@ -41,6 +41,17 @@
   int32_t state_bytes, chunks;
 };
 
+struct alignas(16) SkBankRec {
+  uint8_t head;
+  uint8_t ready;
+  uint8_t busy;
+  uint8_t done;
+  uint32_t deals_consumed;
+  uint32_t plan_ep;
+  uint32_t plan_tag;
+};
+static_assert(sizeof(SkBankRec) == 16, "one dwordx4");
+
 #ifdef __HIPCC__
 #define SK_HD __host__ __device__
 #else
diff --git a/skyjo_rl_amd/csrc/skyjo_record.h b/skyjo_rl_amd/csrc/skyjo_record.h
--- a/skyjo_rl_amd/csrc/skyjo_record.h
+++ b/skyjo_rl_amd/csrc/skyjo_record.h
@@ -78,44 +78,40 @@
   }
 }
 
-__device__ __forceinline__ void bank_advance(const SkParams &P, uint8_t *lp, int g, int head, uint32_t dc) {
-  const uint8_t nh = (uint8_t)((head + 1) % SK_BANK);
-  P.bank_head[g] = nh;
-  LB(H_BANK) = nh;
-  P.deals_consumed[g] = dc + 1;
-  P.done[g] = 0;
+__device__ __forceinline__ void bank_advance(uint8_t *lp, int head, uint4 &r) {
+  const uint32_t nh = (uint32_t)((head + 1) % SK_BANK);
+  r.x = (r.x & 0x00ffff00u) | nh;
+  r.y += 1u;
+  LB(H_BANK) = (uint8_t)nh;
 }
 
-__device__ __forceinline__ bool consume_spare(const SkParams &P, uint8_t *lp, int tile, int lane, int g, int head) {
-  const size_t G = (size_t)P.tiles * SK_TILE;
-  const uint8_t ready = P.spare_ready[(size_t)head * G + g];
-  const uint32_t dc = P.deals_consumed[g];
-  if (!ready) return false;
+__device__ __forceinline__ bool consume_spare(const SkParams &P, uint8_t *lp, int tile, int lane, int g, int head, uint4 r) {
+  if (!BK_READY(r, head)) return false;
   load_spare(P, lp, head, tile, lane);
-  P.spare_ready[(size_t)head * G + g] = 0;
-  bank_advance(P, lp, g, head, dc);
+  r.x &= ~BK_READY_BIT(head);
+  bank_advance(lp, head, r);
+  bank_store(P, g, r);
   return true;
 }
 
 struct SpareRegs {
-  uint32_t dc;
+  uint4 bk;
   int head;
-  uint8_t ready;
 };
 __device__ __forceinline__ void spare_issue(const SkParams &P, uint8_t *lp, uint32_t lds_tile, int tile, int lane, int g, SpareRegs &r) {
-  const size_t G = (size_t)P.tiles * SK_TILE;
   r.head = LB(H_BANK) % SK_BANK;
-  r.ready = P.spare_ready[(size_t)r.head * G + g];
-  r.dc = P.deals_consumed[g];
+  r.bk = bank_load(P, g);
   const uint32_t voff = (uint32_t)(bank_rec16(P, r.head, g) * 16);
   asm volatile("s_waitcnt lgkmcnt(0)" ::: "memory");
   dma_bank_record<false>((const uint8_t *)P.spare, voff, lds_tile, P.L.chunks);
 }
 __device__ __forceinline__ bool spare_commit(const SkParams &P, uint8_t *lp, int g, const SpareRegs &r) {
   sk_vm_drain();
-  if (!r.ready) return false;
-  P.spare_ready[(size_t)r.head * (size_t)P.tiles * SK_TILE + g] = 0;
-  bank_advance(P, lp, g, r.head, r.dc);
+  if (!BK_READY(r.bk, r.head)) return false;
+  uint4 bk = r.bk;
+  bk.x &= ~BK_READY_BIT(r.head);
+  bank_advance(lp, r.head, bk);
+  bank_store(P, g, bk);
   return true;
 }
 
diff --git a/skyjo_rl_amd/csrc/skyjo_step.h b/skyjo_rl_amd/csrc/skyjo_step.h
--- a/skyjo_rl_amd/csrc/skyjo_step.h
+++ b/skyjo_rl_amd/csrc/skyjo_step.h
@@ -3,46 +3,34 @@
 #error "include skyjo_device.h"
 #endif
 
-__device__ __forceinline__ void sk_publish_deals(const SkParams &P, int g) {
-  const size_t G = (size_t)P.tiles * SK_TILE;
-  const int b = P.busy[g];
+__device__ __forceinline__ void sk_publish_deals(const SkParams &P, int g, uint4 &r) {
+  const int b = BK_BUSY(r);
   if (b) {
-    const uint32_t tag = P.plan_tag[g];
+    const uint32_t tag = r.w;
     const uint32_t f = __hip_atomic_load(&P.done_flag[g], __ATOMIC_RELAXED, __HIP_MEMORY_SCOPE_AGENT);
     if ((f & 0x7fffffffu) == tag) {
       SK_FENCE_ACQUIRE(P);
-      if (!P.cancel[g] && f == tag) P.spare_ready[(size_t)(b - 1) * G + g] = 1;
-      P.busy[g] = 0, P.cancel[g] = 0;
-    }
-  }
-}
-__device__ __forceinline__ void sk_plan_deals(const SkParams &P, int g, int lane) {
-  const size_t G = (size_t)P.tiles * SK_TILE;
+      if (!BK_CANCEL(r) && f == tag) r.x |= BK_READY_BIT(b - 1);
+      r.x &= ~(0x00ff0000u | BK_CANCEL_BIT);
+    }
+  }
+}
+__device__ __forceinline__ void sk_bank_put(const SkParams &P, int g, const uint4 &r, const uint4 &was) {
+  if (r.x != was.x || r.z != was.z || r.w != was.w) bank_store(P, g, r);
+}
+__device__ __forceinline__ void sk_plan_deals(const SkParams &P, int g, int lane, uint4 &r) {
   bool need = false, empty = false;
   if (g < P.B) {
-    const uint8_t busy = P.busy[g];
-    const int head = P.bank_head[g] % SK_BANK;
-    const uint32_t consumed = P.deals_consumed[g];
-    uint8_t ready[SK_BANK];
-#pragma unroll
-    for (int k = 0; k < SK_BANK; k++) ready[k] = P.spare_ready[(size_t)k * G + g];
-    bool open = true;
-    int r = 0;
-#pragma unroll
-    for (int k = 0; k < SK_BANK; k++) {
-      uint8_t f = 0;
-#pragma unroll
-      for (int j = 0; j < SK_BANK; j++) f = (head + k) % SK_BANK == j ? ready[j] : f;
-      open = open && f != 0;
-      r += open ? 1 : 0;
-    }
-    need = !busy && r < SK_BANK;
-    empty = need && r == 0;
+    const int busy = BK_BUSY(r);
+    const int head = BK_HEAD(r) % SK_BANK;
+    const int n = bank_ready_run(r);
+    need = !busy && n < SK_BANK;
+    empty = need && n == 0;
     if (need) {
-      P.busy[g] = (uint8_t)(1 + (head + r) % SK_BANK);
-      P.cancel[g] = 0;
-      P.plan_ep[g] = consumed + (uint32_t)r;
-      P.plan_tag[g] = P.plan_new_tag;
+      bank_set_busy(r, 1 + (head + n) % SK_BANK);
+      r.x &= ~BK_CANCEL_BIT;
+      r.z = r.y + (uint32_t)n;
+      r.w = P.plan_new_tag;
     }
   }
   const unsigned long long be = __ballot(empty);
@@ -61,7 +49,7 @@
   for (int p = 0; p < P.L.N; p++) d[p] = P.rewards[(size_t)g * P.L.N + p], d[P.L.N + p] = P.scores[(size_t)g * P.L.N + p];
   uint32_t *m = (uint32_t *)(d + 2 * P.L.N);
   m[0] = P.rng_mode == SKYJO_RNG_MT19937 ? (uint32_t)P.mt_idx[g] : 0u;
-  m[1] = P.done[g];
+  m[1] = bank_get_done(P, g);
 }
 
 __device__ __forceinline__ uint32_t sk_next_tag(uint32_t t) {
@@ -97,7 +85,12 @@
   STAMP_DECL;
   if (!POLICY) tile_load(P, P.state, tile, lane, lp);
   else dma_record<true>((const uint8_t *)P.state, (uint32_t)((((size_t)tile * P.L.chunks) * SK_TILE + lane) * 16), lds_tile, P.L.chunks);
-  if (P.ov_flags & 1u) sk_publish_deals(P, g);
+  if (P.ov_flags & 1u) {
+    const uint4 was = bank_load(P, g);
+    uint4 bk = was;
+    sk_publish_deals(P, g, bk);
+    sk_bank_put(P, g, bk, was);
+  }
   sk_vm_drain();
   HdrRegs h;
   HDR_LOAD(h);
@@ -274,9 +267,12 @@
     }
     STAMP_T(2);
     if (POLICY && cycle_len && it + 1 < iters && (it + 1) % cycle_len == 0) {
-      if (P.busy[g]) (void)wait_deal_done(P, g);
-      sk_publish_deals(P, g);
-      sk_plan_deals(P, g, lane);
+      const uint4 was = bank_load(P, g);
+      uint4 bk = was;
+      if (BK_BUSY(bk)) (void)wait_deal_done(P, g, bk.w);
+      sk_publish_deals(P, g, bk);
+      sk_plan_deals(P, g, lane, bk);
+      sk_bank_put(P, g, bk, was);
       P.plan_new_tag = sk_next_tag(P.plan_new_tag);
       TRACE_WAIT_BEGIN;
       __syncthreads();
@@ -287,11 +283,14 @@
   tile_store_nt(P, P.state, tile, lane, lp);
   if (!POLICY && raw_out && valid) sk_export_raw(P, lp, g, raw_out + (size_t)g * raw_stride);
   if (P.ov_flags & 2u) {
+    const uint4 was = bank_load(P, g);
+    uint4 bk = was;
     if (P.ov_flags & 1u) {
-      if (P.busy[g]) (void)wait_deal_done(P, g);
-      sk_publish_deals(P, g);
-    }
-    sk_plan_deals(P, g, lane);
+      if (BK_BUSY(bk)) (void)wait_deal_done(P, g, bk.w);
+      sk_publish_deals(P, g, bk);
+    }
+    sk_plan_deals(P, g, lane, bk);
+    sk_bank_put(P, g, bk, was);
   }
   if (!POLICY) {
     sk_error_to_host(P, lane);
@@ -387,9 +386,10 @@
   bool want_counted = false;
   tile_load(P, P.state, tile, lane, lp);
   if (want) {
-    const int head = P.bank_head[g] % SK_BANK;
+    const uint4 bk = bank_load(P, g);
+    const int head = BK_HEAD(bk) % SK_BANK;
     bool dealt = true;
-    if (!consume_spare(P, lp, tile, lane, g, head)) dealt = deal_inline(P, lp, fp, g, tile, lane, head);
+    if (!consume_spare(P, lp, tile, lane, g, head, bk)) dealt = deal_inline(P, lp, fp, g, tile, lane, head);
     if (dealt) LB(H_STATUS) = SKYJO_ST_RESET;
     want_counted = dealt;
   }
diff --git a/skyjo_rl_amd/csrc/skyjo_transition.h b/skyjo_rl_amd/csrc/skyjo_transition.h
--- a/skyjo_rl_amd/csrc/skyjo_transition.h
+++ b/skyjo_rl_amd/csrc/skyjo_transition.h
@@ -35,9 +35,8 @@
 #define SK_WAIT_OK 0
 #define SK_WAIT_GAVE_UP 1
 #define SK_WAIT_TIMEOUT 2
-__device__ __forceinline__ int wait_deal_done(const SkParams &P, int g) {
+__device__ __forceinline__ int wait_deal_done(const SkParams &P, int g, const uint32_t tag) {
   uint32_t f = 0;
-  const uint32_t tag = P.plan_tag[g];
   for (int spin = 0; spin < (1 << P.spin_log2); spin++) {
     f = __hip_atomic_load(&P.done_flag[g], __ATOMIC_RELAXED, __HIP_MEMORY_SCOPE_AGENT);
     if ((f & 0x7fffffffu) == tag) break;
@@ -79,32 +78,33 @@
 
 __device__ __forceinline__ void reshuffle_dispatch(const SkParams &P, uint8_t *lp, uint8_t *fp, int g) {
   if (P.rng_mode == SKYJO_RNG_MT19937) {
-    const size_t G = (size_t)P.tiles * SK_TILE;
     uint32_t *mt = P.mt + (size_t)g * 624;
     const int head = LB(H_BANK) % SK_BANK;
-    const int busy = P.busy[g];
-    const bool inflight = busy && !P.cancel[g];
+    uint4 bk = bank_load(P, g);
+    const int busy = BK_BUSY(bk);
+    const bool inflight = busy && !BK_CANCEL(bk);
     bool undo_inflight = false;
     if (inflight) {
-      const int w = wait_deal_done(P, g);
+      const int w = wait_deal_done(P, g, bk.w);
       if (w == SK_WAIT_TIMEOUT) {
         LB(H_FLAGS) |= F_DONE, LB(H_STATUS) = SKYJO_ST_ERROR, LB(H_NDRAW) = 1;
-        P.done[g] = 1;
+        bank_set_done(P, g);
         for (int q = 0; q < P.L.N; q++) P.rewards[(size_t)g * P.L.N + q] = 0.0;
         return;
       }
       undo_inflight = w == SK_WAIT_OK;
-      P.cancel[g] = 1;
+      bk.x |= BK_CANCEL_BIT;
     }
     int packed = P.mt_idx[g];
     if (undo_inflight) packed = mt_rollback(P, mt, g, busy - 1, packed);
     for (int k = SK_BANK - 1; k >= 0; k--) {
       const int slot = (head + k) % SK_BANK;
-      if (P.spare_ready[(size_t)slot * G + g]) {
+      if (BK_READY(bk, slot)) {
         packed = mt_rollback(P, mt, g, slot, packed);
-        P.spare_ready[(size_t)slot * G + g] = 0;
+        bk.x &= ~BK_READY_BIT(slot);
       }
     }
+    bank_store(P, g, bk);
     MtStream<16> r;
     r.open(mt, packed, fp);
     reshuffle_discard(P, lp, r);
@@ -161,7 +161,7 @@
     acc_episode(ap, N, p, d, r, rf);
   }
 #undef SCORE
-  P.done[g] = 1;
+  bank_set_done(P, g);
 }
 
 template <int NP>
@@ -303,7 +303,7 @@
       acc_add(ap, N + p, P.illegal_reward), acc_add(ap, 2 * N + p, P.illegal_reward * P.illegal_reward);
     }
     h.w0 = (h.w0 & 0x0000ffffu) | ((((h.w0 >> 16) & 0xffu) | F_DONE) << 16) | ((uint32_t)SKYJO_ST_ILLEGAL << 24);
-    P.done[g] = 1;
+    bank_set_done(P, g);
     cnt.illegal++;
     return;
   }
@@ -325,7 +325,7 @@
       LB(H_FINISHER) = (uint8_t)p;
       if (NP > 0 && NP < 8) {
         constexpr int NQ = (NP > 0 && NP < 8) ? NP : 1;
-        P.done[g] = 1;
+        bank_set_done(P, g);
         if (pendp) {
 #pragma unroll
           for (int q = 0; q < NQ; q++) *(uint4 *)(pendp + q * 1024) = LQ(sk_pb(P.L, q) >> 4);
```

Measured after the change: 48.17 billion, median of 6. No clear change (+0.3%).
